# fgiral000/gencast-flax-nnx

Hardware: AMD Instinct MI355X
Metric: denoiser-calls/sec (higher is better)
Workload: dtype f16x3 (every product = 3 fp16 MFMAs on hi/lo-split f32 operands: 22-bit products, f32 accumulate; f32 storage); 1 GPU; nano-GenCast DPM-Solver++2S 20-step sample, 2.5deg grid (73x144), 1 ensemble member per GPU, batch 1; dead_call_skipped=True, grid_nodes=10512, mesh_nodes=2562, latent=256, layers=16, heads=4, ffw_hidden=2048, c_in=262, c_out=82, k_hop=8, parallelism=ensemble-dp1, broadcast=none, rccl_ranks=0, precision=f16x3, library_built_from_this_tree=True, launcher=single

## Files before the change

### gencast-flax-nnx_amd/csrc/gc_api.hip

```cpp
#include <dlfcn.h>

#include "gc_handle.h"

using namespace gci;

namespace {

void protect_pending_noise(gc_handle* h) {
  if (h->guard_pending && h->d_noise == h->last_noise) std::swap(h->d_noise, h->d_noise_alt);
}

int check_ready(gc_handle* h) {
  if (!h) return GC_ERR_INVALID_ARGUMENT;
  if (!h->finalized) return fail(h, GC_ERR_STATE, "gc_finalize has not been called");
  return GC_OK;
}

struct Rccl {
  void* lib = nullptr;
  ncclResult_t (*GetUniqueId)(ncclUniqueId*) = nullptr;
  ncclResult_t (*CommInitRank)(ncclComm_t*, int, ncclUniqueId, int) = nullptr;
  ncclResult_t (*CommDestroy)(ncclComm_t) = nullptr;
  ncclResult_t (*CommCount)(const ncclComm_t, int*) = nullptr;
  ncclResult_t (*CommUserRank)(const ncclComm_t, int*) = nullptr;
// ... 2 lines not shown
  const char* (*GetErrorString)(ncclResult_t) = nullptr;
  std::string error;
};

Rccl& rccl() {
  static Rccl r = [] {
    Rccl x;
    const char* override_path = std::getenv("GC_RCCL_LIBRARY");
    for (const char* name : {override_path ? override_path : "/opt/rocm/lib/librccl.so.1", "librccl.so.1", "librccl.so"}) {
      x.lib = dlopen(name, RTLD_NOW | RTLD_GLOBAL);
      if (x.lib) break;
    }
    if (!x.lib) {
      x.error = std::string("cannot load librccl: ") + dlerror();
      return x;
    }
    auto sym = [&](const char* n) {
      void* p = dlsym(x.lib, n);
      if (!p && x.error.empty()) x.error = std::string("librccl lacks ") + n;
      return p;
    };
    x.GetUniqueId = reinterpret_cast<decltype(x.GetUniqueId)>(sym("ncclGetUniqueId"));
    x.CommInitRank = reinterpret_cast<decltype(x.CommInitRank)>(sym("ncclCommInitRank"));
    x.CommDestroy = reinterpret_cast<decltype(x.CommDestroy)>(sym("ncclCommDestroy"));
    x.CommCount = reinterpret_cast<decltype(x.CommCount)>(sym("ncclCommCount"));
    x.CommUserRank = reinterpret_cast<decltype(x.CommUserRank)>(sym("ncclCommUserRank"));
    x.Broadcast = reinterpret_cast<decltype(x.Broadcast)>(sym("ncclBroadcast"));
    x.AllReduce = reinterpret_cast<decltype(x.AllReduce)>(sym("ncclAllReduce"));
    x.GetErrorString = reinterpret_cast<decltype(x.GetErrorString)>(sym("ncclGetErrorString"));
    return x;
  }();
  return r;
}

#define GC_NCCL(h, call)                                                                    \
  do {                                                                                      \
    ncclResult_t r__ = (call);                                                              \
    if (r__ != ncclSuccess) {                                                               \
      (h)->err = std::string(#call) + ": " + rccl().GetErrorString(r__);                    \
      return GC_ERR_COMM;                                                                   \
    }                                                                                       \
  } while (0)

}

static void destroy_impl(gc_handle* h);

extern "C" {

int gc_abi_version(void) { return GC_ABI_VERSION; }

const char* gc_build_info(void) {
#ifndef GC_SOURCE_HASH
#define GC_SOURCE_HASH "unknown"
#endif
  return "libgencast_hip gfx950 f16x3/f32-mfma " __DATE__ " " __TIME__ " src:" GC_SOURCE_HASH;
}

int gc_device_count(void) {
  int n = 0;
  if (hipGetDeviceCount(&n) != hipSuccess) return 0;
  return n;
}

int gc_device_pci_bus_id(int32_t device_id, char* out, int64_t cap) {
  if (!out || cap < 16 || device_id < 0 || device_id >= gc_device_count()) return GC_ERR_INVALID_ARGUMENT;
  out[0] = 0;
  return hipDeviceGetPCIBusId(out, (int)cap, device_id) == hipSuccess ? GC_OK : GC_ERR_HIP;
}

const char* gc_last_error(const gc_handle* h) { return h ? h->err.c_str() : g_create_error.c_str(); }

static void read_switches(gc_handle* h) {
  auto is = [](const char* name, const char* value) { const char* v = std::getenv(name); return v && std::string(v) == value; };
  auto off = [](const char* name) { const char* v = std::getenv(name); return v && *v && std::atoi(v) == 0; };
  auto on = [](const char* name) { const char* v = std::getenv(name); return v && *v == '1'; };
  h->f16x3 = !is("GC_PRECISION", "f32");
  h->use_graphs = !is("GC_TUNE_GRAPH", "0");
  h->m2g_fuse_sum = !off("GC_TUNE_M2G_FUSE_SUM");
  h->embed_cache = !off("GC_TUNE_EMBED_CACHE");
  h->attn_items = !off("GC_TUNE_ATTN_ITEMS");
  h->mlp_pair = !off("GC_TUNE_MLP_PAIR");
  h->edge_terms = !off("GC_TUNE_EDGE_TERMS");
  h->a16 = !off("GC_TUNE_A16");
  h->graph_serialize = on("GC_TUNE_GRAPH_SERIALIZE");
  h->graph_verbose = on("GC_TUNE_GRAPH_VERBOSE");
}

int gc_create(const gc_config* cfg, int device_id, gc_handle** out) {
  return guarded(nullptr, [&]() -> int {
  if (!cfg || !out) { g_create_error = "null argument"; return GC_ERR_INVALID_ARGUMENT; }
  *out = nullptr;
  const gc_config& c = *cfg;
  auto bad = [&](const char* m) { g_create_error = m; return GC_ERR_INVALID_ARGUMENT; };
  if (c.latent_size <= 0 || c.d_model <= 0 || c.num_heads <= 0 || c.ffw_hidden <= 0 ||
      c.num_layers < 0 || c.c_in <= 0 || c.c_out <= 0 || c.batch <= 0)
    return bad("all dimensions must be positive");
  if (c.c_out > c.c_in) return bad("c_out cannot exceed c_in (noisy targets are part of the forcings)");
  if (c.latent_size != c.d_model) return bad("latent_size must equal d_model");
  if (c.d_model % c.num_heads) return bad("num_heads has to divide d_model exactly");
  if (c.noise_num_frequencies <= 0 || c.noise_num_frequencies > 128 || c.noise_hidden <= 0 ||
      c.noise_hidden > 128 || !(c.noise_base_period > 0))
    return bad("noise encoder sizes out of range");
  auto unsup = [&](const char* m) { g_create_error = m; return GC_ERR_UNSUPPORTED; };
  if (c.latent_size != 128 && c.latent_size != 256 && c.latent_size != 512)
    return unsup("latent_size must be 128, 256 or 512 (MFMA column tiling)");
  const int dh = c.d_model / c.num_heads;
  if (dh != 32 && dh != 64 && dh != 128) return unsup("head size must be 32, 64 or 128");
  if (c.num_heads > 8) return unsup("at most 8 heads");
  if (c.ffw_hidden % 128) return unsup("ffw_hidden must be a multiple of 128");
  if (c.c_out > 512) return unsup("c_out must be <= 512");
  int ndev = 0;
  if (hipGetDeviceCount(&ndev) != hipSuccess || ndev == 0) {
    g_create_error = "no HIP device visible (this library has no CPU fallback)";
    return GC_ERR_NO_DEVICE;
  }
  if (device_id < 0 || device_id >= ndev) { g_create_error = "device_id out of range"; return GC_ERR_NO_DEVICE; }
  std::unique_ptr<gc_handle> h(new gc_handle());
  h->cfg = c;
  h->device = device_id;
  hipError_t e = hipSetDevice(device_id);
  if (e == hipSuccess) e = hipStreamCreateWithFlags(&h->stream, hipStreamNonBlocking);
  if (e == hipSuccess) e = hipStreamCreateWithFlags(&h->stream2, hipStreamNonBlocking);
  if (e == hipSuccess) e = hipEventCreate(&h->ev0);
  if (e == hipSuccess) e = hipEventCreate(&h->ev1);
  if (e == hipSuccess) e = hipEventCreateWithFlags(&h->ev_pin, hipEventDisableTiming);
  if (e == hipSuccess) e = hipMalloc((void**)&h->d_nonfinite, sizeof(unsigned));
  if (e == hipSuccess) e = hipMemset(h->d_nonfinite, 0, sizeof(unsigned));
  if (e == hipSuccess) e = hipHostMalloc((void**)&h->h_nonfinite, sizeof(unsigned), hipHostMallocDefault);
  if (e != hipSuccess) {
    g_create_error = hipGetErrorString(e);
    gc_destroy(h.release());
    return GC_ERR_HIP;
  }
  *h->h_nonfinite = 0;
  h->kp = round_up(3 + c.c_in, 32);
  read_switches(h.get());
  build_specs(h.get());
  *out = h.release();
  return GC_OK;
  });
}

void gc_destroy(gc_handle* h) {
  if (!h) return;
  try {
    destroy_impl(h);
  } catch (...) {
  }
}

static void destroy_impl(gc_handle* h) {
  (void)hipSetDevice(h->device);
  if (h->stream) (void)hipStreamSynchronize(h->stream);
  drop_sample_graphs(h);
  if (h->comm) (void)rccl().CommDestroy(h->comm);
  for (gc_handle::CtxSlot& c : h->ctx) {
    if (c.saved) (void)hipEventSynchronize(c.ev_w);
    if (c.read) (void)hipEventSynchronize(c.ev_r);
  }
  for (BufferGroup* g : h->groups) g->free();
  if (h->d_nonfinite) (void)hipFree(h->d_nonfinite);
  for (void* p : {(void*)h->h_nonfinite, (void*)h->pin_cond, (void*)h->pin_noise, (void*)h->pin_forc,
                  (void*)h->pin_lguard})
    if (p) (void)hipHostFree(p);
  if (h->ev_pin) (void)hipEventDestroy(h->ev_pin);
// ... 556 lines not shown
  GC_HIP(h, hipStreamSynchronize(h->stream));
  if (cls >= 0 && h->prof_events.empty()) {
    h->prof_events.resize(2 * 4096);
    for (auto& e : h->prof_events) GC_HIP(h, hipEventCreate(&e));
  }
  h->prof_cls = cls;
  h->prof_used = 0;
  return GC_OK;
}

int gc_profile_set_stride(gc_handle* h, int stride) {
  return guarded(h, [&]() -> int {
  if (!h) return GC_ERR_INVALID_ARGUMENT;
  if (stride < 1) return fail(h, GC_ERR_INVALID_ARGUMENT, "stride must be >= 1");
  h->prof_stride = stride;
  h->prof_seen = 0;
  return GC_OK;
  });
}

int gc_profile_read(gc_handle* h, int32_t* launches, float* total_ms) {
  return guarded(h, [&]() -> int {
  if (!h || !launches || !total_ms) return GC_ERR_INVALID_ARGUMENT;
  GC_HIP(h, hipSetDevice(h->device));
  GC_HIP(h, hipStreamSynchronize(h->stream));
  float tot = 0.f;
  for (size_t i = 0; i + 1 < h->prof_used; i += 2) {
    float ms = 0.f;
    GC_HIP(h, hipEventElapsedTime(&ms, h->prof_events[i], h->prof_events[i + 1]));
    tot += ms;
  }
  *launches = (int32_t)(h->prof_used / 2);
  *total_ms = tot;
  h->prof_used = 0;
  return GC_OK;
  });
}

int gc_algorithmic_work(gc_handle* h, double* flops, double* bytes) {
  return guarded(h, [&]() -> int {
  if (!h || !flops || !bytes) return GC_ERR_INVALID_ARGUMENT;
  if (!h->has_graph) return fail(h, GC_ERR_STATE, "gc_set_graph must be called first");
  const gc_config& c = h->cfg;
  const double B = c.batch, G = h->hg.G * B, M = h->hg.M * B, E1 = h->hg.E1 * B, E2 = h->hg.E2 * B;
  const double L = c.latent_size, D = c.d_model, F = c.ffw_hidden, NL = c.num_layers;
  const double nnz = (double)h->hg.khop_nnz * B;
  double f = 0;
  f += 2 * G * (3 + c.c_in) * L + 2 * G * L * L;
  f += 2 * E1 * 3 * L * L + 2 * E1 * L * L;
  f += 2 * M * 2 * L * L + 2 * M * L * L;
  f += 2 * G * L * L * 2;
  f += NL * (2 * M * D * 3 * D + 2 * M * D * D + 2 * M * D * F * 2 + 4 * nnz * D);
  f += 2 * E2 * 3 * L * L + 2 * E2 * L * L;
  f += 2 * G * 2 * L * L + 2 * G * L * L;
  f += 2 * G * L * L + 2 * G * L * c.c_out;
  f += (h->hidden_layers - 1) * 2.0 * L * L * (G + E1 + M + G + E2 + G + G);
  double params = 0;
  for (const auto& kv : h->specs) {
    double n = 1;
    for (auto d : kv.second) n *= (double)d;
    params += n;
  }
  *bytes = 4.0 * (params + G * (c.c_in + c.c_out) + 2 * G * L + NL * M * D * 10);
  *flops = f;
  return GC_OK;
  });
}

int gc_get_counter(gc_handle* h, const char* name, int64_t* value) {
  return guarded(h, [&]() -> int {
  if (!h) return GC_ERR_INVALID_ARGUMENT;
  if (!name || !value) return fail(h, GC_ERR_INVALID_ARGUMENT, "null argument");
  const std::string n(name);
  if (n == "range_fallbacks") *value = h->range_fallbacks;
  else if (n == "static_embedding_fallbacks") *value = h->static_embedding_fallbacks;
  else if (n == "launches_per_call") *value = h->launches_last_call;
  else if (n == "weights_f16_unsafe") *value = h->weights_f16_unsafe ? 1 : 0;
  else if (n == "fp16_storage") *value = h->last_route.st16 ? 1 : 0;
  else if (n == "split_edge") *value = h->split_edge ? 1 : 0;
  else if (n == "attention_items") *value = h->last_route.att_items;
  else if (n == "m2g_fused_sum") *value = h->last_route.m2g_fused ? 1 : 0;
  else if (n == "embed_cache") *value = h->embed_cache_samples;
  else if (n == "edge_term_samples") *value = h->edge_term_samples;
  else if (n == "edge_term_cache_bytes") *value = h->terms.ready ? h->terms.bytes : 0;
  else if (n == "graph_replays") *value = h->graph_replays;
  else if (n == "graph_captures") *value = h->graph_captures;
  else if (n == "loss_evaluations") *value = h->loss_evaluations;
  else if (n == "loss_device_us") *value = h->loss_device_us;
  else if (n == "ens_scores") *value = h->ens_scores;
  else if (n == "ens_score_device_us") *value = h->ens_score_device_us;
  else if (n == "ens_invalid_points") *value = h->ens_invalid_points;
  else if (n == "spec_calls") *value = h->spec_calls;
  else if (n == "spec_device_us") *value = h->spec_device_us;
  else if (n == "spec_invalid_columns") *value = h->spec_invalid_columns;
  else if (n == "ens_event_calls") *value = h->evt_calls;
  else if (n == "ens_event_device_us") *value = h->evt_device_us;
  else if (n == "ens_event_invalid_points") *value = h->evt_invalid_points;
  else if (n == "ens_derive_calls") *value = h->drv_calls;
  else if (n == "ens_derive_device_us") *value = h->drv_device_us;
  else if (n == "ens_order_calls") *value = h->ord_calls;
  else if (n == "ens_order_device_us") *value = h->ord_device_us;
  else if (n == "ens_order_invalid_points") *value = h->ord_invalid_points;
  else if (n == "ens_clim_calls") *value = h->clim_calls;
  else if (n == "ens_clim_device_us") *value = h->clim_device_us;
  else if (n == "ens_clim_invalid_points") *value = h->clim_invalid_points;
  else if (n == "ens_energy_calls") *value = h->en_calls;
  else if (n == "ens_energy_device_us") *value = h->en_device_us;
  else if (n == "ens_energy_invalid_points") *value = h->en_invalid_points;
  else if (n == "ens_variogram_calls") *value = h->vg_calls;
  else if (n == "ens_variogram_device_us") *value = h->vg_device_us;
  else if (n == "ens_tail_calls") *value = h->tail_calls;
  else if (n == "ens_tail_device_us") *value = h->tail_device_us;
  else if (n == "ens_tail_invalid_points") *value = h->tail_invalid_points;
  else if (n == "ens_region_calls") *value = h->reg_calls;
  else if (n == "ens_region_device_us") *value = h->reg_device_us;
  else if (n == "ens_feature_calls") *value = h->feat_calls;
  else if (n == "ens_feature_device_us") *value = h->feat_device_us;
  else if (n == "ens_region_invalid_points") *value = h->reg_invalid_points;
  else if (n == "ens_fss_calls") *value = h->fss_calls;
  else if (n == "ens_fss_device_us") *value = h->fss_device_us;
  else if (n == "ens_window_pushes") *value = h->win_pushes;
  else if (n == "ens_window_emits") *value = h->win_emits;
  else if (n == "ens_window_device_us") *value = h->win_device_us;
  else if (n == "ens_window_ring_bytes")
    *value = (int64_t)((size_t)h->win_ring_L * (((size_t)(h->win_ring_M + 1) * h->hg.G * h->cfg.batch * h->cfg.c_out + 3) / 4 * 4) * sizeof(float));
  else if (n == "noise_stream") *value = (int64_t)h->nz_stream;
  else if (n == "device_allocations") {
    *value = 0;
    for (const BufferGroup* g : h->groups) *value += (int64_t)g->ptrs.size();
  }
  else return fail(h, GC_ERR_INVALID_ARGUMENT, "unknown counter: " + n);
  return GC_OK;
  });
}

int gc_noise_set_tables(gc_handle* h, int32_t n_lat, int32_t n_lon, int32_t lmax, const float* legendre,
                        const float* cos_table, const float* sin_table) {
  return guarded(h, [&]() -> int {
  if (!h) return GC_ERR_INVALID_ARGUMENT;
  if (!h->has_graph) return fail(h, GC_ERR_STATE, "gc_set_graph must be called first");
  if (!legendre || !cos_table || !sin_table) return fail(h, GC_ERR_INVALID_ARGUMENT, "null argument");
  if (n_lat < 2 || n_lon < 2 || lmax < 1 || (int64_t)n_lat * n_lon != h->hg.G)
    return fail(h, GC_ERR_INVALID_ARGUMENT, "n_lat * n_lon must equal the number of grid nodes");
  const int N = h->cfg.batch * h->cfg.c_out;
  GC_HIP(h, hipSetDevice(h->device));
  int rc;
  const size_t L = (size_t)lmax;
  if ((rc = dev_upload(h, &h->d_nz_leg, std::vector<float>(legendre, legendre + L * n_lat * L)))) return rc;
  if ((rc = dev_upload(h, &h->d_nz_cos, std::vector<float>(cos_table, cos_table + (size_t)n_lon * L)))) return rc;
  if ((rc = dev_upload(h, &h->d_nz_sin, std::vector<float>(sin_table, sin_table + (size_t)n_lon * L)))) return rc;
  if ((rc = dev_alloc(h, &h->d_nz_coef, 2 * L * L * N + 4))) return rc;
  if ((rc = dev_alloc(h, &h->d_nz_f, 2 * L * n_lat * N))) return rc;
  h->nz_L = lmax; h->nz_lat = n_lat; h->nz_lon = n_lon;
  return GC_OK;
  });
}

int gc_noise_seed(gc_handle* h, uint64_t seed, uint64_t stream) {
  return guarded(h, [&]() -> int {
  if (!h) return GC_ERR_INVALID_ARGUMENT;
  if (h->guard_pending) {
    GC_HIP(h, hipSetDevice(h->device));
    int rc = resolve_guard(h);
    if (rc) return rc;
  }
  h->nz_key = seed;
// ... 465 lines not shown
```

### gencast-flax-nnx_amd/csrc/gc_forward.hip

```cpp
#include "gc_handle.h"

namespace gci {

template <class To, class From>
static const To& a16_view(const From& v) {
  static_assert(sizeof(To) == sizeof(From), "argument struct mismatch between the two kernel builds");
  return reinterpret_cast<const To&>(v);
}

Route make_route(const gc_handle* h) {
  const int D = h->cfg.d_model, F = h->cfg.ffw_hidden;
  Route r;
  r.f16 = h->f16x3 && !h->weights_f16_unsafe && !h->in_fallback;
  r.x32 = !r.f16 && h->f32_ws;
  const bool streams = r.f16 || r.x32;
  r.ffw_slabs = streams ? h->ffw_fused_slabs : 0;
  r.st16 = h->feat16 && h->a16 && r.f16 && D % 128 == 0 && D <= 512 &&
           (h->ffw_fused_slabs > 0 || (F % 128 == 0 && (F / h->ffw2_splits) % 128 == 0));
  r.v2 = r.f16 && r.ws(3 * D, D, 1);
  r.att_items = (h->att_n_items > 0 && r.ws(3 * D, D, 1) && h->attn_splits == 1 && D <= 512) ? h->att_n_items : 0;
  r.fuse_row = streams && D % 128 == 0 && D <= 512;
  r.node_ws = r.f16;
  r.split_edge = h->split_edge;
  r.try_pair = h->mlp_pair && h->hidden_layers == 1;
  r.m2g_fused = h->m2g_fuse_sum && h->hg.m2g_tri && h->hidden_layers == 1 && streams;
  r.embed_cache = h->embed_cache_live && h->embed_cache_ready && !h->feat16 && h->hidden_layers == 1 && streams;
  r.edge_terms = h->embed_cache_live && h->terms.ready && edge_terms_possible(h) && r.f16;
  return r;
}

bool edge_terms_possible(const gc_handle* h) {
  return h->edge_terms && h->f16x3 && !h->weights_f16_unsafe && !h->in_fallback && !h->feat16 && h->hidden_layers == 1 &&
         h->cfg.latent_size == 256 && h->cfg.batch == 1 && h->hg.m2g_tri;
}

static gc::Segment seg(const float* ptr, const int* index, const float* affine, int width, int ld, int bcast) {
  gc::Segment s;
  s.ptr = ptr; s.index = index; s.affine = affine; s.width = width; s.ld = ld; s.bcast = bcast;
  return s;
}

struct MlpCall {
  gc::Segment seg[3] = {};
  gc::AddTerm add[3] = {};
  int nseg = 0, nadd = 0, rows = 0, B = 1, ldo = 0;
  bool ln = true, cond = true;
  const float* residual = nullptr;
  float* out = nullptr;
  bool round_out = true;
  bool seg0_f32 = false, out_f32 = false;
  bool tri = false;
  MlpCall& segments(std::initializer_list<gc::Segment> l) { for (const auto& s : l) seg[nseg++] = s; return *this; }
  MlpCall& add_terms(std::initializer_list<gc::AddTerm> l) { for (const auto& t : l) add[nadd++] = t; return *this; }
};
static MlpCall mlp_call(std::initializer_list<gc::Segment> segs, int rows, int B, float* out, int ldo,
                        const float* residual = nullptr) {
  MlpCall c;
  c.rows = rows; c.B = B; c.out = out; c.ldo = ldo; c.residual = residual;
  return c.segments(segs);
}

static int build_mlp_args(gc_handle* h, const DevMlp& w, const MlpCall& c, gc::MlpArgs* out_args) {
  const Route& r = h->route;
  gc::MlpArgs& a = *out_args;
  a = gc::MlpArgs{};
  a.nseg = c.nseg; a.nadd = c.nadd;
  std::copy(c.seg, c.seg + c.nseg, a.seg);
  std::copy(c.add, c.add + c.nadd, a.add);
  a.rows = c.rows; a.B = c.B; a.hidden = h->cfg.latent_size;
  a.f16 = r.f16 ? 1 : 0;
  const Weight& w1 = c.nadd ? w.w1e : w.w1;
  a.w1t = pick(w1, r, Form::Staged); a.ldw1 = w1.ld; a.b1 = w.b1;
  a.w2t = pick(w.w2, r, Form::Staged); a.b2 = w.b2;
  if (r.f16 || r.x32) {
    a.w1f = pick(w1, r, Form::Streaming); a.k1f = w1.kf;
    a.w2f = pick(w.w2, r, Form::Streaming); a.ones = h->d_ones; a.zeros = h->d_zeros;
    a.f32w = r.x32 ? 1 : 0;
  }
  a.n_out = w.n_out; a.n_out_pad = w.n_out_pad; a.do_ln = c.ln ? 1 : 0;
  a.cond = (c.cond && w.cond_off >= 0) ? (h->cond_cur ? h->cond_cur : h->d_cond) + w.cond_off : nullptr;
  a.cond_stride = h->cond_total;
  a.residual = c.residual; a.out = c.out; a.ldo = c.ldo;
  a.round16 = h->feat16 ? 1 : 0;
  a.round_out = (h->feat16 && c.round_out) ? 1 : 0;
  a.a16 = r.st16 ? 1 : 0;
  a.seg0_f32 = c.seg0_f32 ? 1 : 0;
  a.out_f32 = c.out_f32 ? 1 : 0;
  a.tri = c.tri ? 1 : 0;
  if (c.tri && !gc::mlp_runs_weight_streaming(a))
    return fail(h, GC_ERR_INTERNAL, "the triple-sum epilogue exists in the weight-streaming MLP kernel only");
  return GC_OK;
}

static int enqueue_mlp(gc_handle* h, const gc::MlpArgs& a) {
  return launch(h, gc::KC_MLP, [&] {
    return a.a16 ? gc_a16::launch_mlp(h->stream, a16_view<gc_a16::MlpArgs>(a)) : gc::launch_mlp(h->stream, a);
  });
}
static int enqueue_mlp_pair(gc_handle* h, const gc::MlpArgs& a, const gc::MlpArgs& b) {
  return launch(h, gc::KC_MLP, [&] {
    return a.a16 ? gc_a16::launch_mlp_pair(h->stream, a16_view<gc_a16::MlpArgs>(a), a16_view<gc_a16::MlpArgs>(b))
                 : gc::launch_mlp_pair(h->stream, a, b);
  });
}
static int enqueue_gemm_ws(gc_handle* h, int cls, const gc::GemmArgs& ga, int mt, int splits, int epi) {
  return launch(h, cls, [&] {
    return ga.a16 ? gc_a16::launch_gemm_ws(h->stream, cls, a16_view<gc_a16::GemmArgs>(ga), mt, splits, epi)
                  : gc::launch_gemm_ws(h->stream, cls, ga, mt, splits, epi);
  });
}
static int enqueue_gemm_rowop(gc_handle* h, int cls, const gc::GemmArgs& ga, const gc::RowFuse& rf) {
  return launch(h, cls, [&] {
    return ga.a16 ? gc_a16::launch_gemm_rowop(h->stream, cls, a16_view<gc_a16::GemmArgs>(ga), a16_view<gc_a16::RowFuse>(rf))
                  : gc::launch_gemm_rowop(h->stream, cls, ga, rf);
  });
}
static int enqueue_ffw_fused(gc_handle* h, const gc::FfwArgs& fa) {
  return launch(h, gc::KC_GEMM_FFW1, [&] {
    return fa.a16 ? gc_a16::launch_ffw_fused(h->stream, a16_view<gc_a16::FfwArgs>(fa)) : gc::launch_ffw_fused(h->stream, fa);
  });
}

static int run_mlp_one(gc_handle* h, const DevMlp& w, const MlpCall& c) {
  gc::MlpArgs a{};
  if (int rc = build_mlp_args(h, w, c, &a)) return rc;
  return enqueue_mlp(h, a);
}

static int run_mlp(gc_handle* h, const DevMlp& w, const MlpCall& c) {
  if (w.pre.empty()) return run_mlp_one(h, w, c);
  if (c.nadd || c.tri || !h->d_mlp_tmp[0]) return fail(h, GC_ERR_INTERNAL, "hidden_layers >= 2: unsupported MLP form");
  const int L = h->cfg.latent_size;
  auto handed = [&](MlpCall m, size_t buf) {
    m.nseg = 0; m.seg0_f32 = true;
    return m.segments({seg(h->d_mlp_tmp[buf & 1], nullptr, nullptr, L, L, 0)});
  };
  MlpCall lead = c;
  lead.ln = lead.cond = lead.round_out = false; lead.residual = nullptr; lead.ldo = L; lead.out_f32 = true;
  for (size_t i = 0; i < w.pre.size(); ++i) {
    lead.out = h->d_mlp_tmp[i & 1];
    if (int rc = run_mlp_one(h, w.pre[i], i ? handed(lead, i - 1) : lead)) return rc;
  }
  return run_mlp_one(h, w, handed(c, w.pre.size() - 1));
}

int pick_ws_mt(int rows, int n, int splits) {
  const int panels = (n / 128) * splits;
  return ((rows + 63) / 64) * panels >= 400 ? 2 : 1;
}

bool build_attention_items(const gc::HostGraph& g, std::vector<int>* items, std::vector<int>* tiles) {
  const int n = g.n_tiles;
  tiles->assign((size_t)2 * n, 0);
  std::vector<std::vector<int>> lists(8);
  int slot = 0, any_cut = 0;
  for (int x = 0; x < 8; ++x) {
    const int t0 = (int)((long long)n * x / 8), t1 = (int)((long long)n * (x + 1) / 8), ng = t1 - t0;
    if (ng < 32) return false;
    if (ng >= 64) return false;
    const int n_cut = ng % 32;
    if (n_cut > 16) return false;
    any_cut += n_cut;
    std::vector<char> cut(ng, 0);
    for (int k = 0; k < n_cut; ++k) cut[(int)(((2LL * k + 1) * ng) / (2LL * n_cut))] = 1;
    std::vector<int>& it = lists[x];
    std::vector<int> order;
    for (int i = 0; i < ng; ++i) {
      const int t = t0 + i;
      if (cut[i]) { order.push_back(t); continue; }
      it.insert(it.end(), {t, g.tile_chunk_start[t], g.tile_chunk_start[t + 1], -1});
    }
// ... 80 lines not shown

static gc::GemmArgs mesh_gemm_args(const gc_handle* h, const float* a, int lda, bool ws) {
  gc::GemmArgs ga{};
  ga.a = a; ga.lda = lda; ga.a_f32 = 1; ga.rows = h->hg.M * h->cfg.batch;
  ga.round16 = h->feat16 ? 1 : 0; ga.a16 = h->route.st16 ? 1 : 0; ga.f32w = (ws && h->route.x32) ? 1 : 0;
  return ga;
}
static void merge_attention_partials(const gc_handle* h, gc::GemmArgs* ga) {
  const int D = h->cfg.d_model, H = h->cfg.num_heads;
  ga->att_po = h->d_apart_o; ga->att_pml = h->d_apart_ml; ga->att_B = h->cfg.batch; ga->att_H = H; ga->att_DH = D / H;
  if (h->attn_splits > 1) ga->att_S = h->attn_splits;
  else ga->att_tiles = h->d_att_tiles;
}
static int mesh_gemm(gc_handle* h, int cls, const float* a, int lda, const Weight& w, int n, int k, int splits,
                     const float* bias, int act, float* out, int ldo, int epi, bool att_merge = false) {
  const Route& r = h->route;
  const bool ws = r.ws(n, k, splits);
  gc::GemmArgs ga = mesh_gemm_args(h, a, lda, ws);
  ga.wt = pick(w, r, ws ? Form::Streaming : Form::Staged); ga.ldw = k; ga.n = n; ga.k_slice = k / splits;
  ga.bias = bias; ga.act = act; ga.out = out; ga.ldo = ldo;
  if (att_merge) merge_attention_partials(h, &ga);
  if (ws) return enqueue_gemm_ws(h, cls, ga, att_merge ? 1 : pick_ws_mt(ga.rows, n, splits), splits, epi);
  return launch(h, cls, [&] { return gc::launch_gemm(h->stream, cls, ga, splits, epi, r.f16); });
}

int forward(gc_handle* h, float sigma_scalar, const float* cond_ready) {
  const gc_config& c = h->cfg;
  const gc::HostGraph& g = h->hg;
  const int B = c.batch, L = c.latent_size, D = c.d_model, F = c.ffw_hidden;
  hipStream_t s = h->stream;
  int rc;
  const float* cond = cond_ready ? cond_ready : h->d_cond;
  h->cond_cur = cond;
  const int cs = h->cond_total;
  const int64_t launches0 = h->launch_count;
  const Route& r = h->route = h->last_route = make_route(h);

  if (!cond_ready && (rc = launch(h, gc::KC_COND, [&] {
         return gc::launch_cond(s, sigma_scalar < 0 ? h->d_sigma : nullptr, sigma_scalar, B, h->d_nw0t,
                                h->d_nb0, h->d_nw1t, h->d_nb1, c.noise_num_frequencies, c.noise_hidden,
                                c.noise_base_period, h->d_wc_all, h->d_bc_all, cs, h->d_condvec,
                                h->d_cond);
       })))
    return rc;

  {
    MlpCall embed = r.embed_cache ? mlp_call({seg(h->d_xn, nullptr, nullptr, h->nwp, h->nwp, 0)}, g.G * B, B, h->d_g0, L)
                                  : mlp_call({seg(h->d_xp, nullptr, nullptr, h->kp, h->kp, 0)}, g.G * B, B, h->d_g0, L);
    embed.seg0_f32 = true;
    if (r.embed_cache) embed.add_terms({{h->d_pstat, nullptr}});
    if ((rc = run_mlp(h, r.embed_cache ? h->g2m_embed_grid_n : h->g2m_embed_grid, embed))) return rc;
  }
  const size_t ML = (size_t)g.M * L;
  if (r.edge_terms && (h->term_slot < 0 || !h->terms.ready))
    return fail(h, GC_ERR_INTERNAL, "edge terms: the forward has no slot of the cache");
  const float* const m0 = r.edge_terms ? h->terms.m0 + h->term_slot * ML : h->d_m0;
  h->m0_cur = m0;
  if (!r.edge_terms && (rc = launch(h, gc::KC_PACK, [&] {
         return gc::launch_affine_rows(s, h->d_m0_hat, cond + h->g2m_embed_mesh.cond_off, cs, g.M, B, L,
                                       h->d_m0, h->feat16, r.st16);
       })))
    return rc;
  if (r.edge_terms && (rc = node_gemm(h, h->d_g0, g.G * B, h->g2m_edge.w1snd, h->d_pg))) return rc;
  const MlpCall edge = r.edge_terms
                           ? edge_terms_call(h, h->terms.T1 + (size_t)h->term_slot * g.E1 * L, g.E1, h->d_g2m_snd, h->d_g2m_rcv,
                                             h->d_pg, h->terms.Pm + h->term_slot * ML, h->d_e1)
                           : edge_call(h, h->d_e0_hat, cond + h->g2m_embed_edge.cond_off, g.E1, h->d_g2m_snd, h->d_g2m_rcv,
                                       h->d_g0, h->d_m0, h->d_pg, h->d_pm, h->d_e1);
  const MlpCall node = mlp_call({seg(h->d_g0, nullptr, nullptr, L, L, 0)}, g.G * B, B, h->d_g1, L, h->d_g0);
  gc::MlpArgs ea{}, na{};
  bool paired = false;
  if (r.try_pair) {
    if ((rc = build_mlp_args(h, h->g2m_edge, edge, &ea)) || (rc = build_mlp_args(h, h->g2m_grid, node, &na))) return rc;
    paired = gc::mlp_pair_supported(ea, na);
  }
  if (r.split_edge && (rc = edge_node_products(h, h->g2m_edge, h->d_g0, g.G * B, h->d_pg, h->d_m0, g.M * B, h->d_pm)))
    return rc;
  if ((rc = paired ? enqueue_mlp_pair(h, ea, na) : run_mlp(h, h->g2m_edge, edge))) return rc;
  if ((rc = launch(h, gc::KC_SEGSUM, [&] {
         return gc::launch_segsum(s, h->d_e1, h->d_g2m_ptr, h->d_g2m_eid, g.M, g.E1, B, L, h->d_agg1, h->feat16, r.st16,
                                  h->g2m_agg_norm);
       })))
    return rc;
  if ((rc = run_mlp(h, h->g2m_mesh, mlp_call({seg(m0, nullptr, nullptr, L, L, 0), seg(h->d_agg1, nullptr, nullptr, L, L, 0)},
                                             g.M * B, B, h->d_x, L, m0))))
    return rc;
  if (!paired && (rc = run_mlp(h, h->g2m_grid, node))) return rc;

  const int MB = g.M * B;
  const int n_layers = (h->debug_layer_limit >= 0 && h->debug_layer_limit < c.num_layers)
                           ? h->debug_layer_limit : c.num_layers;
  const float* pend_bias = nullptr;
  int pend_slabs = 0;
  auto rowop = [&](const float* bias, int slabs, int cond_off, float* hout) {
    return launch(h, gc::KC_ROWOP, [&] {
      return gc::launch_rowop(s, h->d_x, bias, h->d_part, slabs, MB, D, B, cond + cond_off, cs, hout, 0, h->feat16, r.st16);
    });
  };
  auto stop_here = [&](int i, int phase) { return h->debug_stop_layer == i && h->debug_stop_phase == phase; };
  const int* att_items = r.att_items ? h->d_att_items : nullptr;
  for (int i = 0; i < n_layers; ++i) {
    const DevLayer& ly = h->layers[i];
    if ((rc = rowop(pend_bias, pend_slabs, ly.cond_attn, h->d_h))) return rc;
    if (stop_here(i, 0)) return GC_OK;
    if (r.v2) {
      gc::GemmArgs ga = mesh_gemm_args(h, h->d_h, D, true);
      ga.wt = pick(ly.wqkv, r, Form::Streaming); ga.ldw = D; ga.n = 3 * D; ga.k_slice = D;
      ga.out = h->d_qkv; ga.ldo = r.st16 ? D : 3 * D;
      ga.kv16 = h->d_kv16; ga.kv_d = D;
      if ((rc = enqueue_gemm_ws(h, gc::KC_GEMM_QKV, ga, pick_ws_mt(MB, 3 * D, 1), 1, 3))) return rc;
      if (stop_here(i, 1)) return GC_OK;
      if ((rc = launch(h, gc::KC_ATTN, [&] {
             return gc::launch_attention_v2(s, h->d_qkv, h->d_kv16, h->d_att, h->d_apart_o, h->d_apart_ml, g.M, B, D,
                                            c.num_heads, h->attn_splits, h->d_tile_start, h->d_union, h->d_mask,
                                            g.n_tiles, h->max_tile_chunks, h->feat16, r.st16, att_items, r.att_items);
           })))
        return rc;
    } else {
      if ((rc = mesh_gemm(h, gc::KC_GEMM_QKV, h->d_h, D, ly.wqkv, 3 * D, D, 1, nullptr, 0, h->d_qkv, 3 * D, 0))) return rc;
      if (stop_here(i, 1)) return GC_OK;
      if ((rc = launch(h, gc::KC_ATTN, [&] {
             return gc::launch_attention(s, h->d_qkv, h->d_att, h->d_apart_o, h->d_apart_ml, g.M, B, D,
                                         c.num_heads, h->attn_splits, false, h->d_tile_start, h->d_union,
                                         h->d_mask, g.n_tiles, h->feat16, att_items, r.att_items);
           })))
        return rc;
    }
    if (r.fuse_row) {
      gc::GemmArgs ga = mesh_gemm_args(h, h->d_att, D, true);
      ga.wt = pick(ly.wo, r, Form::Streaming); ga.ldw = D; ga.n = D; ga.k_slice = D;
      if (h->attn_splits > 1 || r.att_items) merge_attention_partials(h, &ga);
      gc::RowFuse rf{h->d_x, ly.bo, cond + ly.cond_ffw, cs, B, h->d_h, h->feat16 ? 1 : 0};
      if ((rc = enqueue_gemm_rowop(h, gc::KC_GEMM_OUT, ga, rf))) return rc;
    } else {
      if ((rc = mesh_gemm(h, gc::KC_GEMM_OUT, h->d_att, D, ly.wo, D, D, h->out_splits, nullptr, 0, h->d_part, D, 1, h->attn_splits > 1)))
        return rc;
      if ((rc = rowop(ly.bo, h->out_splits, ly.cond_ffw, h->d_h))) return rc;
    }
    if (stop_here(i, 2)) return GC_OK;
    if (r.ffw_slabs > 0) {
      gc::FfwArgs fa{h->d_h, MB, (int)D, (int)F, pick(ly.w1, r, Form::Streaming), ly.b1, pick(ly.w2, r, Form::Streaming),
                     h->d_part, h->feat16 ? 1 : 0, r.st16 ? 1 : 0};
      fa.f32w = r.x32 ? 1 : 0;
      if ((rc = enqueue_ffw_fused(h, fa))) return rc;
    } else {
      if ((rc = mesh_gemm(h, gc::KC_GEMM_FFW1, h->d_h, D, ly.w1, F, D, 1, ly.b1, 1, h->d_u, F, 0))) return rc;
      if ((rc = mesh_gemm(h, gc::KC_GEMM_FFW2, h->d_u, F, ly.w2, D, F, h->ffw2_splits, nullptr, 0, h->d_part, D, 1))) return rc;
    }
    pend_bias = ly.b2;
    pend_slabs = r.ffw_slabs > 0 ? r.ffw_slabs : h->ffw2_splits;
  }
  if ((rc = rowop(pend_bias, pend_slabs, h->cond_final, h->d_m2))) return rc;

  if ((r.split_edge || r.edge_terms) && (rc = edge_node_products(h, h->m2g_edge, h->d_m2, g.M * B, h->d_pm, h->d_g1, g.G * B, h->d_pg)))
    return rc;
  if ((rc = run_m2g_edge(h, cond, r.m2g_fused))) return rc;
  if (!r.m2g_fused && (rc = launch(h, gc::KC_SEGSUM, [&] {
         return gc::launch_segsum(s, h->d_f1, h->d_m2g_ptr, h->d_m2g_eid, g.G, g.E2, B, L, h->d_agg2, h->feat16, r.st16);
       })))
    return rc;
  if ((rc = run_mlp(h, h->m2g_grid, mlp_call({seg(h->d_g1, nullptr, nullptr, L, L, 0), seg(h->d_agg2, nullptr, nullptr, L, L, 0)},
                                             g.G * B, B, h->d_g2, L, h->d_g1))))
    return rc;
  MlpCall dec = mlp_call({seg(h->d_g2, nullptr, nullptr, L, L, 0)}, g.G * B, B, h->d_y, c.c_out);
  dec.ln = dec.cond = false; dec.out_f32 = true;
  if ((rc = run_mlp(h, h->m2g_dec, dec))) return rc;
  h->launches_last_call = h->launch_count - launches0;
  return GC_OK;
}

int compute_static_embeddings(gc_handle* h) {
  const gc::HostGraph& hg = h->hg;
  const int L = h->cfg.latent_size;
  const struct { const DevMlp& w; const float* in; int items; float* out; } embeds[] = {
      {h->g2m_embed_mesh, h->d_mesh_struct16, hg.M, h->d_m0_hat},
      {h->g2m_embed_edge, h->d_e1_struct16, hg.E1, h->d_e0_hat},
      {h->m2g_embed_edge, h->d_e2_struct16, hg.E2, h->d_f0_hat}};
  if (int rc = drop_edge_terms(h)) return rc;
  auto run = [&]() -> int {
    h->route = make_route(h);
    for (const auto& e : embeds) {
      MlpCall c = mlp_call({seg(e.in, nullptr, nullptr, 32, 32, 1)}, e.items, 1, e.out, L);
      c.cond = c.round_out = false; c.seg0_f32 = c.out_f32 = true;
      if (int rc = run_mlp(h, e.w, c)) return rc;
    }
    return GC_OK;
  };
  if (int rc = run()) return rc;
  GC_HIP(h, hipStreamSynchronize(h->stream));
  if (!h->route.f16 || h->feat16) return GC_OK;
  const unsigned before = *h->h_nonfinite;
  for (const auto& e : embeds)
    if (int rc = launch(h, gc::KC_PACK, [&] { return gc::launch_finite_check(h->stream, e.out, (size_t)e.items * L, h->d_nonfinite); }))
      return rc;
  GC_HIP(h, hipMemcpyAsync(h->h_nonfinite, h->d_nonfinite, sizeof(unsigned), hipMemcpyDeviceToHost, h->stream));
  GC_HIP(h, hipStreamSynchronize(h->stream));
  const unsigned hits = *h->h_nonfinite - before;
  if (!hits) return GC_OK;
  h->nonfinite_seen += hits;
  ++h->static_embedding_fallbacks;
  h->in_fallback = true;
  const int rc = run();
  h->in_fallback = false;
  if (rc) return rc;
  GC_HIP(h, hipStreamSynchronize(h->stream));
  return GC_OK;
}

int drop_edge_terms(gc_handle* h) {
  if (h->terms.sigmas.empty() && h->term_allocs.ptrs.empty()) return GC_OK;
  if (!h->term_allocs.ptrs.empty()) {
    GC_HIP(h, hipStreamSynchronize(h->stream));
    drop_sample_graphs(h);
    h->term_allocs.free();
  }
  h->terms = gc_handle::EdgeTerms{};
  h->term_slot = -1;
  return GC_OK;
}

int ensure_edge_terms(gc_handle* h, const std::vector<float>& call_sigma) {
  if (!edge_terms_possible(h)) return GC_OK;
  gc_handle::EdgeTerms& t = h->terms;
  if (t.sigmas.size() == call_sigma.size() &&
      !std::memcmp(t.sigmas.data(), call_sigma.data(), call_sigma.size() * sizeof(float)))
    return GC_OK;
  if (int rc = drop_edge_terms(h)) return rc;
  t.sigmas = call_sigma;
  std::vector<float> distinct;
  for (float sg : call_sigma) {
    size_t k = 0;
    while (k < distinct.size() && std::memcmp(&distinct[k], &sg, sizeof(float))) ++k;
    if (k == distinct.size()) distinct.push_back(sg);
    t.call_slot.push_back((int)k);
  }
  const gc::HostGraph& g = h->hg;
  const gc_config& c = h->cfg;
  const size_t L = c.latent_size, n = distinct.size();
  const size_t per_slot = ((size_t)g.E1 + g.E2 + 2 * (size_t)g.M) * L;
  t.bytes = (int64_t)(n * per_slot * sizeof(float));
  if (n == 0 || n > (size_t)gc::kMaxSigmaList || t.bytes > h->edge_term_cap_mb * (int64_t)(1 << 20) ||
      n * (size_t)c.batch * h->cond_total > h->cond_all_cap) {
    t.bytes = 0;
    return GC_OK;
  }
  int rc;
  BufferGroup* own = &h->term_allocs;
  if ((rc = dev_alloc(h, &t.T1, n * g.E1 * L, own)) || (rc = dev_alloc(h, &t.T2, n * g.E2 * L, own)) ||
      (rc = dev_alloc(h, &t.m0, n * g.M * L, own)) || (rc = dev_alloc(h, &t.Pm, n * g.M * L, own)))
// ... 31 lines not shown
```

### gencast-flax-nnx_amd/csrc/gc_handle.h

```cpp
#pragma once
#include <hip/hip_runtime.h>

#include <algorithm>
#include <array>
#include <cmath>
#include <cstdio>
#include <cstdlib>
#include <cstring>
#include <map>
#include <memory>
#include <mutex>
#include <string>
#include <vector>

#include <rccl/rccl.h>

#include "../../include/gencast_hip.h"
#include "../../include/gencast_hip_debug.h"
#include "gc_graph.h"
#include "gc_kernels.h"

namespace gci {

inline int round_up(int v, int m) { return (v + m - 1) / m * m; }

struct Route {
  bool f16 = false;
  bool x32 = false;
  bool st16 = false;
  int ffw_slabs = 0;
  bool v2 = false;
  int att_items = 0;
  bool fuse_row = false;
  bool node_ws = false;
  bool m2g_fused = false;
  bool split_edge = false;
  bool try_pair = false;
  bool embed_cache = false;
  bool edge_terms = false;
  bool ws(int n, int k, int splits) const { return (f16 || x32) && n % 128 == 0 && (k / splits) % 128 == 0; }
};

struct Weight {
  float* t = nullptr;
  float* s = nullptr;
  float* f = nullptr;
  float* x = nullptr;
  int ld = 0, kf = 0;
};
enum class Form { Staged, Streaming };
inline const float* pick(const Weight& w, const Route& r, Form form) {
  if (form == Form::Streaming) return r.x32 ? w.x : w.f;
  return r.f16 ? w.s : w.t;
}

struct DevMlp {
  Weight w1, w2;
  Weight w1e, w1snd, w1rcv;
  float *b1 = nullptr, *b2 = nullptr;
  int n_out = 0, n_out_pad = 0;
  int cond_off = -1;
  std::vector<DevMlp> pre;
};

struct DevLayer {
  Weight wqkv, wo, w1, w2;
  float *bo = nullptr, *b1 = nullptr, *b2 = nullptr;
  int cond_attn = -1, cond_ffw = -1;
};

struct BufferGroup {
  std::vector<void*> ptrs;
  explicit BufferGroup(std::vector<BufferGroup*>& of_handle) { of_handle.push_back(this); }
  BufferGroup(const BufferGroup&) = delete;
  void free() {
    for (void* p : ptrs) (void)hipFree(p);
    ptrs.clear();
  }
  hipError_t drop(hipStream_t s) {
    const hipError_t e = hipStreamSynchronize(s);
    if (e == hipSuccess) free();
    return e;
  }
};

struct Event {
  hipEvent_t e = nullptr;
  explicit Event(std::vector<Event*>& of_handle) { of_handle.push_back(this); }
  Event(const Event&) = delete;
  hipError_t ensure(bool timing = false) {
    return e ? hipSuccess : timing ? hipEventCreate(&e) : hipEventCreateWithFlags(&e, hipEventDisableTiming);
  }
};

struct Bracket {
  Event e0, e1;
  explicit Bracket(std::vector<Event*>& of_handle) : e0(of_handle), e1(of_handle) {}
  hipError_t ensure() {
    const hipError_t e = e0.ensure(true);
    return e != hipSuccess ? e : e1.ensure(true);
  }
  hipError_t begin(hipStream_t s) { return hipEventRecord(e0.e, s); }
  hipError_t end(hipStream_t s) { return hipEventRecord(e1.e, s); }
  hipError_t microseconds(int64_t* us) {
    float ms = 0.f;
    const hipError_t e = hipEventElapsedTime(&ms, e0.e, e1.e);
    *us = (int64_t)(ms * 1000.0f);
    return e;
  }
};

}

struct gc_handle {
  std::vector<gci::BufferGroup*> groups;
  std::vector<gci::Event*> events;
  gc_config cfg{};
  int device = 0;
  hipStream_t stream = nullptr;
  hipStream_t stream2 = nullptr;
  std::string err;
  bool has_graph = false, finalized = false, has_slots = false, has_cond = false, has_noise = false;
  bool finalized_weights = false;
  gc::HostGraph hg;

  std::map<std::string, std::vector<int64_t>> specs;
  std::map<std::string, std::vector<float>> weights;
  gci::BufferGroup allocs{groups}, weight_allocs{groups}, cache_allocs{groups};

  int *d_g2m_snd = nullptr, *d_g2m_rcv = nullptr, *d_m2g_snd = nullptr, *d_m2g_rcv = nullptr;
  int *d_g2m_ptr = nullptr, *d_g2m_eid = nullptr, *d_m2g_ptr = nullptr, *d_m2g_eid = nullptr;
  int *d_tile_start = nullptr, *d_union = nullptr;
  int *d_att_items = nullptr, *d_att_tiles = nullptr;
  int att_n_items = 0;
  unsigned* d_mask = nullptr;
  float *d_grid_struct = nullptr, *d_mesh_struct16 = nullptr, *d_e1_struct16 = nullptr,
        *d_e2_struct16 = nullptr;

  gci::DevMlp g2m_embed_grid, g2m_embed_mesh, g2m_embed_edge, g2m_edge, g2m_mesh, g2m_grid;
  gci::DevMlp m2g_embed_edge, m2g_edge, m2g_grid, m2g_dec;
  std::vector<gci::DevLayer> layers;
  int cond_final = -1;
  int cond_total = 0;
  std::map<std::string, std::pair<int, int>> cond_sites;
  float *d_nw0t = nullptr, *d_nb0 = nullptr, *d_nw1t = nullptr, *d_nb1 = nullptr;
  float *d_wc_all = nullptr, *d_bc_all = nullptr;

  float *d_m0_hat = nullptr, *d_e0_hat = nullptr, *d_f0_hat = nullptr;

  int kp = 0;
  float *d_sigma = nullptr, *d_condvec = nullptr, *d_cond = nullptr;
  float* d_cond_all = nullptr;
  size_t cond_all_cap = 0;
  const float* cond_cur = nullptr;
  float *d_feats = nullptr, *d_xp = nullptr, *d_g0 = nullptr, *d_g1 = nullptr, *d_m0 = nullptr,
        *d_x = nullptr, *d_e1 = nullptr, *d_agg1 = nullptr, *d_qkv = nullptr, *d_att = nullptr,
        *d_u = nullptr, *d_m2 = nullptr, *d_f1 = nullptr, *d_agg2 = nullptr, *d_g2 = nullptr,
        *d_y = nullptr, *d_h = nullptr, *d_part = nullptr, *d_apart_o = nullptr, *d_apart_ml = nullptr,
        *d_pg = nullptr, *d_pm = nullptr;
  bool mlp_pair = true;
  bool embed_cache = true;
  bool embed_cache_ready = false;
  bool embed_cache_live = false;
  int nwp = 0;
  float *d_xn = nullptr, *d_pstat = nullptr;
  float *w1st_t = nullptr, *w1st_s = nullptr;
  gci::DevMlp g2m_embed_grid_n;
  std::vector<int> h_slots;
  int64_t embed_cache_samples = 0;
  bool m2g_fuse_sum = true;
  struct EdgeTerms {
    bool ready = false;
    std::vector<float> sigmas;
    std::vector<int> call_slot;
    float *T1 = nullptr, *T2 = nullptr, *m0 = nullptr, *Pm = nullptr;
    int64_t bytes = 0;
  };
  bool edge_terms = true;
  int64_t edge_term_cap_mb = 4096;
  EdgeTerms terms;
  gci::BufferGroup term_allocs{groups};
  int term_slot = -1;
  const float* m0_cur = nullptr;
  int64_t edge_term_samples = 0;
  float *d_ones = nullptr, *d_zeros = nullptr;
  int hidden_layers = 1;
  float* d_mlp_tmp[2] = {nullptr, nullptr};
  float *d_feats2 = nullptr, *d_ro_a = nullptr, *d_ro_b = nullptr, *d_ro_forc = nullptr;
  int *d_ro_kind = nullptr, *d_ro_src = nullptr, *d_ro_sidx = nullptr;
  int ro_nforc = -1, ro_forc_cap = 0;
  bool has_sample = false;
  int max_tile_chunks = 0;
  int ffw_fused_slabs = 0;
  void* d_kv16 = nullptr;
  bool f32_ws = true;
  bool split_edge = false;
  int attn_splits = 1, out_splits = 1, ffw2_splits = 1;
  gci::Route route;
  gci::Route last_route;
  bool a16 = true;
  bool attn_items = true;
  bool graph_serialize = false;
  bool graph_verbose = false;
  int* d_slots = nullptr;
  float *d_sx = nullptr, *d_sden = nullptr, *d_smid = nullptr, *d_noise = nullptr;
  float *d_noise_alt = nullptr, *last_noise = nullptr;
  float* d_stash = nullptr;
  hipEvent_t ev_stash = nullptr;
  bool has_stash = false;

  int nz_L = 0, nz_lat = 0, nz_lon = 0;
  float *d_nz_leg = nullptr, *d_nz_cos = nullptr, *d_nz_sin = nullptr, *d_nz_coef = nullptr, *d_nz_f = nullptr;
  unsigned long long nz_key = 0, nz_stream = 0;
  std::vector<float> churn_rates;
  float churn_inflation = 1.0f;

  bool has_loss_weights = false, has_targets = false, has_denoised = false;
  int loss_groups = 0;
  float *d_lw_node = nullptr, *d_lw_chan = nullptr, *d_lw_group = nullptr;
  int* d_l_group = nullptr;
  float *d_targets = nullptr, *d_lx = nullptr, *d_lden = nullptr;
  double* d_lpart = nullptr;
  float *d_lsig = nullptr, *d_lloss = nullptr, *d_lpg = nullptr;
  int loss_cap = 0;
  unsigned* pin_lguard = nullptr;
  int64_t loss_evaluations = 0, loss_device_us = 0;

  gci::BufferGroup ens_allocs{groups};
  int ens_members = 0;
  std::vector<char> ens_filled;
  float* d_ens = nullptr;
  double* d_ens_part = nullptr;
  unsigned* d_ens_hpart = nullptr;
  double* d_ens_sums = nullptr;
  unsigned long long* d_ens_hist = nullptr;
  float *d_ens_w = nullptr, *d_ens_truth = nullptr;
  float *d_ens_mean = nullptr, *d_ens_var = nullptr;
  bool has_ens_w = false, has_ens_truth = false, has_ens_fields = false;
  gci::Event ev_ens_free{events}, ev_ens_done{events};
  gci::Bracket ens_time{events};
  int64_t ens_scores = 0, ens_score_device_us = 0, ens_invalid_points = 0;
  std::vector<int32_t> ens_state_src;
  int* d_ens_state_src = nullptr;

  gci::BufferGroup ctx_allocs{groups};
  int ctx_slots = 0;
  float* d_ctx = nullptr;
  struct CtxSlot {
    bool saved = false;
    bool read = false;
    hipEvent_t ev_w = nullptr, ev_r = nullptr;
  };
  std::vector<CtxSlot> ctx;

  gci::BufferGroup spec_allocs{groups};
  gci::BufferGroup spec_work_allocs{groups};
  int sp_L = 0, sp_lat = 0, sp_lon = 0;
  int sp_sets = 0;
  float *d_sp_q = nullptr, *d_sp_tab = nullptr;
  float* d_sp_field = nullptr;
  double* d_sp_F = nullptr;
  double* d_sp_coef = nullptr;
  double* d_sp_out = nullptr;
  unsigned* d_sp_flags = nullptr;
  gci::Bracket spec_time{events};
  int64_t spec_calls = 0, spec_device_us = 0, spec_invalid_columns = 0;

// ... 73 lines not shown
  double* d_en_part = nullptr;
  unsigned* d_en_ipart = nullptr;
  double* d_en_out = nullptr;
  unsigned long long* d_en_outc = nullptr;
  gci::Bracket en_time{events};
  int64_t en_calls = 0, en_device_us = 0, en_invalid_points = 0;
  gci::BufferGroup vg_allocs{groups};
  bool vg_set = false;
  int vg_O = 0, vg_pk = 0, vg_n_lat = 0, vg_n_lon = 0;
  int* d_vg_offs = nullptr;
  double* d_vg_part = nullptr;
  unsigned* d_vg_cpart = nullptr;
  double* d_vg_out = nullptr;
  unsigned long long* d_vg_outc = nullptr;
  gci::Bracket vg_time{events};
  int64_t vg_calls = 0, vg_device_us = 0;

  gci::BufferGroup tail_allocs{groups};
  gci::BufferGroup tail_work_allocs{groups};
  int tail_T = 0;
  unsigned tail_dir_up = 0;
  int tail_work_T = 0;
  float* d_tail_thr = nullptr;
  double* d_tail_part = nullptr;
  unsigned* d_tail_cpart = nullptr;
  double* d_tail_out = nullptr;
  unsigned long long* d_tail_outc = nullptr;
  gci::Bracket tail_time{events};
  int64_t tail_calls = 0, tail_device_us = 0, tail_invalid_points = 0;

  gci::BufferGroup reg_allocs{groups};
  int reg_R = 0;
  int reg_listed = 0, reg_blocks = 0;
  std::vector<int> reg_plan;
  int reg_dev_M = 0;
  int* d_reg_plan = nullptr;
  double* d_reg_part = nullptr;
  unsigned* d_reg_hpart = nullptr;
  double* d_reg_sums = nullptr;
  unsigned long long* d_reg_hist = nullptr;
  gci::Bracket reg_time{events};
  int64_t reg_calls = 0, reg_device_us = 0, reg_invalid_points = 0;

  gci::BufferGroup feat_allocs{groups};
  gci::BufferGroup feat_work_allocs{groups};
  bool feat_set = false;
  bool feat_listed = false;
  int feat_c_src = 0, feat_n_lat = 0, feat_n_lon = 0, feat_max = 0, feat_list_M = 0;
  double* d_feat_depth = nullptr;
  int* d_feat_tab = nullptr;
  unsigned char* d_feat_work = nullptr;
  size_t feat_work_bytes = 0;
  int *d_feat_count = nullptr, *d_feat_node = nullptr;
  float* d_feat_value = nullptr;
  gci::Bracket feat_time{events};
  gci::Event ev_feat_src{events};
  int64_t feat_calls = 0, feat_device_us = 0;

  gci::BufferGroup fss_allocs{groups};
  gci::BufferGroup fss_work_allocs{groups};
  int fss_S = 0;
  int fss_n_lat = 0, fss_n_lon = 0;
  std::vector<int32_t> fss_rlat;
  int *d_fss_rlat = nullptr, *d_fss_rlon = nullptr;
  unsigned* d_fss_roww = nullptr;
  uint2* d_fss_work = nullptr;
  double* d_fss_part = nullptr;
  double* d_fss_out = nullptr;
  size_t fss_work_len = 0, fss_part_len = 0, fss_out_len = 0;
  gci::Bracket fss_time{events};
  int64_t fss_calls = 0, fss_device_us = 0;

  struct SampleGraph {
    std::vector<float> sigmas;
    int skip_dead = 1;
    const float* noise = nullptr;
    bool feat16 = false;
    gci::Route route;
    hipGraph_t graph = nullptr;
    hipGraphExec_t exec = nullptr, exec2 = nullptr;
    hipEvent_t done[2] = {nullptr, nullptr};
    int next = 0;
    int calls = 0;
    int64_t launches_per_call = 0, launches = 0;
    uint64_t last_use = 0;
  };
  bool use_graphs = true;
  std::vector<SampleGraph> sample_graphs;
  uint64_t graph_clock = 0;
  int64_t graph_replays = 0, graph_captures = 0;
  int debug_layer_limit = -1;
  int debug_stop_layer = -1, debug_stop_phase = -1;
  bool f16x3 = true;
  float g2m_agg_norm = 0.f;
  bool feat16 = false;
  bool weights_f16_unsafe = false;
  bool in_fallback = false;
  unsigned* d_nonfinite = nullptr;
  unsigned* h_nonfinite = nullptr;
  unsigned nonfinite_seen = 0;
  int64_t range_fallbacks = 0;
  int64_t static_embedding_fallbacks = 0;
  bool guard_pending = false;
  std::vector<float> last_sigmas;
  int last_skip_dead = 1;
  unsigned long long last_stream0 = 0;
  int64_t launches_last_call = 0, launch_count = 0;
  float *pin_cond = nullptr, *pin_noise = nullptr, *pin_forc = nullptr;
  size_t pin_forc_cap = 0;
  hipEvent_t ev_pin = nullptr;
  ncclComm_t comm = nullptr;
  int comm_rank = 0, comm_world = 1;
  double* d_comm_scalar = nullptr;

  int prof_cls = -1;
  int prof_stride = 1;
  unsigned prof_seen = 0;
  std::vector<hipEvent_t> prof_events;
  size_t prof_used = 0;
  hipEvent_t ev0 = nullptr, ev1 = nullptr;
};

namespace gci {

#define GC_HIP(h, call)                                                                     \
  do {                                                                                      \
    hipError_t e__ = (call);                                                                \
    if (e__ != hipSuccess) {                                                                \
      (h)->err = std::string(#call) + ": " + hipGetErrorString(e__);                        \
      return GC_ERR_HIP;                                                                    \
    }                                                                                       \
  } while (0)

inline int fail(gc_handle* h, int code, const std::string& msg) {
  h->err = msg;
  return code;
}

template <typename T>
int dev_alloc(gc_handle* h, T** p, size_t count, BufferGroup* owner = nullptr) {
  void* q = nullptr;
  GC_HIP(h, hipMalloc(&q, std::max<size_t>(count, 1) * sizeof(T)));
  (owner ? owner : &h->allocs)->ptrs.push_back(q);
  *p = reinterpret_cast<T*>(q);
  return GC_OK;
}

template <typename T>
int dev_upload(gc_handle* h, T** p, const std::vector<T>& v, BufferGroup* owner = nullptr) {
  int rc = dev_alloc(h, p, v.size(), owner);
  if (rc) return rc;
  if (!v.empty()) GC_HIP(h, hipMemcpy(*p, v.data(), v.size() * sizeof(T), hipMemcpyHostToDevice));
  return GC_OK;
}

template <typename F>
int launch(gc_handle* h, int cls, F&& f) {
  ++h->launch_count;
  bool prof = (h->prof_cls == cls) && (h->prof_used + 2 <= h->prof_events.size());
  if (prof && h->prof_stride > 1) prof = ((h->prof_seen++ % (unsigned)h->prof_stride) == 0);
  if (prof) GC_HIP(h, hipEventRecord(h->prof_events[h->prof_used], h->stream));
  hipError_t e = f();
  if (e != hipSuccess) {
    h->err = std::string("launch ") + gc::kernel_class_name(cls) + ": " + hipGetErrorString(e);
    return GC_ERR_HIP;
  }
  if (prof) {
// ... 71 lines not shown
```

### gencast-flax-nnx_amd/csrc/gc_kernels.hip

```cpp
#include "gc_kernels.h"

#include <algorithm>
#include <atomic>
#include <type_traits>

#include <math.h>
#include <stdlib.h>

#ifdef GC_TU_A16
#define GC_TU_NS gc_a16
#else
#define GC_TU_NS gc
#endif
namespace GC_TU_NS {
#ifdef GC_TU_A16
constexpr bool kTuA16 = true;
#else
constexpr bool kTuA16 = false;
#endif

#include "gc_dev_common.inc"


struct DynLdsOnce {
// ... 424 lines not shown
  return v;
}

template <int NT, int R>
__device__ __forceinline__ void ws_ring_fill(f32x4 (&wh)[R][NT], f32x4 (&wl)[R][NT], const float* wf,
                                             size_t ct_stride, int steps_total) {
#pragma unroll
  for (int j = 0; j < R; ++j) {
    const int sn = j < steps_total ? j : steps_total - 1;
#pragma unroll
    for (int nt = 0; nt < NT; ++nt) {
      wh[j][nt] = ld4(wf + nt * ct_stride + (size_t)sn * 512);
      wl[j][nt] = ld4(wf + nt * ct_stride + (size_t)sn * 512 + 256);
    }
  }
}

template <int MT, int NT, int R, int J0, bool A16 = false, bool F32 = false>
__device__ __forceinline__ void ws_quad(f32x16 (&acc)[MT][NT], f32x16 (&acc2)[MT][NT], f32x4 (&wh)[R][NT],
                                        f32x4 (&wl)[R][NT], const float* a_row, int mt_stride, int kstep0,
                                        const float* wf, size_t ct_stride, int& s, int steps_total) {
#pragma unroll
  for (int j = 0; j < 4; ++j) {
    const int kk = kstep0 + j;
    const int off = F32 ? kk * 16 : (kk >> 1) * 32 + (kk & 1) * 8;
#pragma unroll
    for (int mt = 0; mt < MT; ++mt) {
      if constexpr (F32) {
        const f32x4 a0 = ld4(a_row + mt * mt_stride + off), a1 = ld4(a_row + mt * mt_stride + off + 4);
#pragma unroll
        for (int e = 0; e < 4; ++e)
#pragma unroll
          for (int nt = 0; nt < NT; ++nt) acc[mt][nt] = mfma32(wh[J0 + j][nt][e], a0[e], acc[mt][nt]);
#pragma unroll
        for (int e = 0; e < 4; ++e)
#pragma unroll
          for (int nt = 0; nt < NT; ++nt) acc[mt][nt] = mfma32(wl[J0 + j][nt][e], a1[e], acc[mt][nt]);
        continue;
      }
      const f32x4 ah = ld4(a_row + mt * mt_stride + off);
      f32x4 al;
      if constexpr (!A16) al = ld4(a_row + mt * mt_stride + off + 16);
#pragma unroll
      for (int nt = 0; nt < NT; ++nt) acc2[mt][nt] = mfma16(wl[J0 + j][nt], ah, acc2[mt][nt]);
#pragma unroll
      for (int nt = 0; nt < NT; ++nt) acc[mt][nt] = mfma16(wh[J0 + j][nt], ah, acc[mt][nt]);
      if constexpr (!A16) {
#pragma unroll
        for (int nt = 0; nt < NT; ++nt) acc2[mt][nt] = mfma16(wh[J0 + j][nt], al, acc2[mt][nt]);
      }
    }
    __builtin_amdgcn_sched_barrier(0);
    int sn = s + R;
    if (sn >= steps_total) sn = steps_total - 1;
#pragma unroll
    for (int nt = 0; nt < NT; ++nt) {
      wh[J0 + j][nt] = ld4(wf + nt * ct_stride + (size_t)sn * 512);
      wl[J0 + j][nt] = ld4(wf + nt * ct_stride + (size_t)sn * 512 + 256);
    }
    ++s;
    __builtin_amdgcn_sched_barrier(0);
  }
}

__device__ __forceinline__ void ln_accumulate(const f32x4& y, float& s1, float& s2) {
#pragma unroll
  for (int e = 0; e < 4; ++e) {
    s1 += y[e];
    s2 = __builtin_fmaf(y[e], y[e], s2);
  }
}
__device__ __forceinline__ void ln_finish(float s1, float s2, float inv_n, float& mean, float& rstd) {
  mean = s1 * inv_n;
  const float var = fmaxf(__builtin_fmaf(-mean, mean, s2 * inv_n), 0.f);
  rstd = 1.0f / sqrtf(var + 1e-6f);
}
__device__ __forceinline__ f32x4 ln_affine(const f32x4& y, float mean, float rstd, const f32x4& sc, const f32x4& of) {
  f32x4 r;
#pragma unroll
  for (int e = 0; e < 4; ++e) r[e] = __builtin_fmaf((y[e] - mean) * rstd, sc[e], of[e]);
  return r;
}

template <int NT1, int WM, int NWC>
constexpr int mlp_ws_occ() { return NWC >= 8 ? (NT1 == 1 ? 4 : 2) : ((WM >= 2 || NT1 >= 4) ? 1 : 2); }
template <int NT1, int NT2, int MT, int WM, int NWC, int NW2, int OCC, bool A16, bool F32, bool TERMS = false>
__device__ __forceinline__ void gc_mlp_ws_body(const MlpArgs& a, const int bid) {
  static_assert(!(A16 && F32), "one or the other");
  static_assert(!TERMS || (!A16 && !F32 && (NT1 * 32 * NWC) % 256 == 0 && (32 * MT) % (4 * NWC) == 0), "terms form: f16x3, whole 1 KB rows per wave");
  extern __shared__ __attribute__((aligned(16))) float smem[];
  constexpr int HID = NT1 * 32 * NWC, NPAD = NT2 * 32 * NW2, BM = 32 * MT * WM, NTHR = 64 * NWC * WM;
  constexpr int KC = BM >= 128 ? 64 : 128, LDA = KC + 4, LDH = HID + 4, LDY = NPAD + 4;
  constexpr int PPR = KC / 4;
  constexpr int RSTEP = NTHR / PPR;
  constexpr int AP = BM / RSTEP;
  constexpr int R1 = (OCC < 4 && (NT1 * MT <= 2 || (NT1 >= 4 && MT == 1))) ? 8 : 4;
  constexpr int R2 = (OCC < 4 && (NT2 * MT <= 2 || (NT1 >= 4 && NT2 * MT <= 4))) ? 8 : 4;
  int* srcoff = reinterpret_cast<int*>(smem);
  int* srcb = srcoff + 3 * BM;
  int* addoff = srcb + BM;
  float* region = smem + 6 * BM;

  const int tid = threadIdx.x;
  const int wave_all = tid >> 6, lane = tid & 63, r = lane & 31, hh = lane >> 5;
  const int wave = wave_all % NWC, wrow = (wave_all / NWC) * (MT * 32);
  const int row0 = bid * BM;
  constexpr int TPB = BM / 3;
  const int tri = a.tri;
  const int unit0 = bid * TPB, units = a.rows / 3;
  const int w0 = a.seg[0].width, w1 = a.nseg > 1 ? a.seg[1].width : 0, w2 = a.nseg > 2 ? a.seg[2].width : 0;
  const int ktot = w0 + w1 + w2, kpad = a.k1f;

  const float *p0 = a.seg[0].ptr, *p1 = a.seg[1].ptr, *p2 = a.seg[2].ptr;
  const float *f0 = a.seg[0].affine, *f1 = a.nseg > 1 ? a.seg[1].affine : nullptr,
              *f2 = a.nseg > 2 ? a.seg[2].affine : nullptr;
  if constexpr (TERMS) {
    const int *ax0 = a.add[0].index, *ax1 = a.add[1].index, *ax2 = a.add[2].index;
    for (int idx = tid; idx < a.nadd * BM; idx += NTHR) {
      const int t = idx / BM, i = idx - t * BM;
      int grow = row0 + i;
      if (grow >= a.rows) grow = a.rows - 1;
      int item = grow / a.B, b = grow - item * a.B;
      if (tri) {
        const int j = i / 3;
        int u = unit0 + j;
        if (u >= units) u = units - 1;
        const int gi = u / a.B;
        b = u - gi * a.B;
        item = 3 * gi + (i - 3 * j);
      }
      const int* ax = pick3(t, ax0, ax1, ax2);
      srcoff[idx] = ((ax ? ax[item] : item) * a.B + b) * HID;
    }
  }
  if constexpr (!TERMS) {
    const int *ix0 = a.seg[0].index, *ix1 = a.seg[1].index, *ix2 = a.seg[2].index;
    const int bc0 = a.seg[0].bcast, bc1 = a.seg[1].bcast, bc2 = a.seg[2].bcast;
    const int ld0 = a.seg[0].ld, ld1 = a.seg[1].ld, ld2 = a.seg[2].ld;
    for (int idx = tid; idx < a.nseg * BM; idx += NTHR) {
      const int sgi = idx / BM, i = idx - sgi * BM;
      int grow = row0 + i;
      if (grow >= a.rows) grow = a.rows - 1;
      int item = grow / a.B, b = grow - item * a.B;
      if (tri) {
        const int j = i / 3;
        int u = unit0 + j;
        if (u >= units) u = units - 1;
        const int gi = u / a.B;
        b = u - gi * a.B;
        item = 3 * gi + (i - 3 * j);
      }
      const int* ix = pick3(sgi, ix0, ix1, ix2);
      const int bc = pick3(sgi, bc0, bc1, bc2);
      const int ld = pick3(sgi, ld0, ld1, ld2);
      int srow = ix ? ix[item] : item;
      if (!bc) srow = srow * a.B + b;
      srcoff[idx] = srow * ld;
      if (sgi == 0) srcb[i] = b;
    }
    const int* ax0 = a.add[0].index;
    const int* ax1 = a.add[1].index;
    for (int idx = tid; idx < a.nadd * BM; idx += NTHR) {
      const int t = idx / BM, i = idx - t * BM;
      int grow = row0 + i;
      if (grow >= a.rows) grow = a.rows - 1;
      int item = grow / a.B, b = grow - item * a.B;
      if (tri) {
        const int j = i / 3;
        int u = unit0 + j;
        if (u >= units) u = units - 1;
        const int gi = u / a.B;
// ... 279 lines not shown
        f32x4 y3[3][CG];
#pragma unroll
        for (int sl = 0; sl < 3; ++sl)
#pragma unroll
          for (int j = 0; j < CG; ++j) {
            const int c = 4 * lane + 256 * j;
            f32x4 y = {0.f, 0.f, 0.f, 0.f};
            if (c < NPAD) {
              y = ld4(Ybuf + (3 * jt + sl) * LDY + c);
#pragma unroll
              for (int e = 0; e < 4; ++e)
                if (c + e >= n) y[e] = 0.f;
            }
            y3[sl][j] = y;
          }
        float mean3[3] = {0.f, 0.f, 0.f}, rstd3[3] = {1.f, 1.f, 1.f};
        if (a.do_ln) {
          float s1[3], s2[3];
#pragma unroll
          for (int sl = 0; sl < 3; ++sl) {
            s1[sl] = 0.f;
            s2[sl] = 0.f;
#pragma unroll
            for (int j = 0; j < CG; ++j) ln_accumulate(y3[sl][j], s1[sl], s2[sl]);
          }
#pragma unroll
          for (int o = 32; o > 0; o >>= 1)
#pragma unroll
            for (int sl = 0; sl < 3; ++sl) {
              s1[sl] += __shfl_xor(s1[sl], o);
              s2[sl] += __shfl_xor(s2[sl], o);
            }
#pragma unroll
          for (int sl = 0; sl < 3; ++sl) ln_finish(s1[sl], s2[sl], inv_n, mean3[sl], rstd3[sl]);
        }
#pragma unroll
        for (int j = 0; j < CG; ++j) {
          const int c = 4 * lane + 256 * j;
          if (c >= n) continue;
          f32x4 sc = scpre[j], of = ofpre[j];
          if (a.cond && a.B != 1) {
            const float* cs = a.cond + (size_t)(u % a.B) * a.cond_stride;
            sc = ld4(cs + c);
            of = ld4(cs + n + c);
          }
          f32x4 t = r16_c<RND>(ln_affine(y3[0][j], mean3[0], rstd3[0], sc, of));
          t += r16_c<RND>(ln_affine(y3[1][j], mean3[1], rstd3[1], sc, of));
          t += r16_c<RND>(ln_affine(y3[2][j], mean3[2], rstd3[2], sc, of));
          t = r16_c<RND>(t);
          if (A16 && !a.out_f32) sth4(as_h16(a.out) + (size_t)u * a.ldo + c, t);
          else st4(a.out + (size_t)u * a.ldo + c, t);
        }
      }
    });
    return;
  }
#pragma unroll
  for (int j = 0; j < CG; ++j) {
    const int c = 4 * lane + 256 * j;
#pragma unroll
    for (int rr = 0; rr < RW; ++rr) {
      const int orow = row0 + rbase + rr;
      f32x4 rs = {0.f, 0.f, 0.f, 0.f};
      if (a.residual && orow < a.rows && c < n) {
        if constexpr (A16) {
          if (vec_io) {
            rs = ldh4(as_h16(a.residual) + (size_t)orow * n + c);
          } else {
#pragma unroll
            for (int e = 0; e < 4; ++e)
              if (c + e < n) rs[e] = (float)as_h16(a.residual)[(size_t)orow * n + c + e];
          }
        } else if (vec_io) {
          rs = ld4(a.residual + (size_t)orow * n + c);
        } else {
#pragma unroll
          for (int e = 0; e < 4; ++e)
            if (c + e < n) rs[e] = a.residual[(size_t)orow * n + c + e];
        }
      }
      rv[rr][j] = rs;
    }
  }
  __syncthreads();
#pragma unroll
  for (int rr = 0; rr < RW; ++rr) {
#pragma unroll
    for (int j = 0; j < CG; ++j) {
      const int c = 4 * lane + 256 * j;
      f32x4 y = {0.f, 0.f, 0.f, 0.f};
      if (c < NPAD) {
        y = ld4(Ybuf + (rbase + rr) * LDY + c);
#pragma unroll
        for (int e = 0; e < 4; ++e)
          if (c + e >= n) y[e] = 0.f;
      }
      yv[rr][j] = y;
    }
  }
  float mean[RW], rstd[RW];
  if (a.do_ln) {
    float s1[RW], s2[RW];
#pragma unroll
    for (int rr = 0; rr < RW; ++rr) {
      s1[rr] = 0.f;
      s2[rr] = 0.f;
#pragma unroll
      for (int j = 0; j < CG; ++j) ln_accumulate(yv[rr][j], s1[rr], s2[rr]);
    }
#pragma unroll
    for (int o = 32; o > 0; o >>= 1)
#pragma unroll
      for (int rr = 0; rr < RW; ++rr) {
        s1[rr] += __shfl_xor(s1[rr], o);
        s2[rr] += __shfl_xor(s2[rr], o);
      }
#pragma unroll
    for (int rr = 0; rr < RW; ++rr) ln_finish(s1[rr], s2[rr], inv_n, mean[rr], rstd[rr]);
  } else {
#pragma unroll
    for (int rr = 0; rr < RW; ++rr) {
      mean[rr] = 0.f;
      rstd[rr] = 1.f;
    }
  }
  with_flag(a.round_out, [&](auto rc) __attribute__((always_inline)) {
  constexpr bool RND = decltype(rc)::value;
#pragma unroll
  for (int j = 0; j < CG; ++j) {
    const int c = 4 * lane + 256 * j;
    if (c >= n) continue;
    const f32x4 sc1 = scpre[j], of1 = ofpre[j];
#pragma unroll
    for (int rr = 0; rr < RW; ++rr) {
      const int orow = row0 + rbase + rr;
      if (orow >= a.rows) break;
      f32x4 sc = sc1, of = of1;
      if (a.cond && !(a.B == 1 && vec_io)) {
        const float* cs = a.cond + (size_t)(orow % a.B) * a.cond_stride;
#pragma unroll
        for (int e = 0; e < 4; ++e)
          if (c + e < n) {
            sc[e] = cs[c + e];
            of[e] = cs[n + c + e];
          }
      }
      const f32x4 v = r16_c<RND>(r16_c<RND>(ln_affine(yv[rr][j], mean[rr], rstd[rr], sc, of)) + rv[rr][j]);
      if (A16 && !a.out_f32) {
        if (vec_io) {
          sth4(as_h16(a.out) + (size_t)orow * a.ldo + c, v);
        } else {
#pragma unroll
          for (int e = 0; e < 4; ++e)
            if (c + e < n) as_h16(a.out)[(size_t)orow * a.ldo + c + e] = (_Float16)v[e];
        }
      } else if (vec_io) {
        st4(a.out + (size_t)orow * a.ldo + c, v);
      } else {
#pragma unroll
        for (int e = 0; e < 4; ++e)
          if (c + e < n) a.out[(size_t)orow * a.ldo + c + e] = v[e];
      }
    }
  }
  });
}

template <int NT1, int NT2, int MT, int WM, int NWC = 4, int NW2 = NWC,
          int OCC = mlp_ws_occ<NT1, WM, NWC>() , bool A16 = false,
          bool F32 = false, bool TERMS = false>
__global__ __launch_bounds__(64 * NWC * WM, OCC) void gc_mlp_ws_kernel(MlpArgs a) {
  gc_mlp_ws_body<NT1, NT2, MT, WM, NWC, NW2, OCC, A16, F32, TERMS>(a, (int)blockIdx.x);
}

template <int NT1, int NT2, int MT, int WM, int NWC = 4, int NW2 = NWC,
          int OCC = mlp_ws_occ<NT1, WM, NWC>(), bool A16 = false, bool F32 = false, bool TERMS_A = false >
__global__ __launch_bounds__(64 * NWC * WM, OCC) void gc_mlp_ws_pair_kernel(MlpArgs a, MlpArgs b, int na) {
  if ((int)blockIdx.x < na) gc_mlp_ws_body<NT1, NT2, MT, WM, NWC, NW2, OCC, A16, F32, TERMS_A>(a, (int)blockIdx.x);
  else gc_mlp_ws_body<NT1, NT2, MT, WM, NWC, NW2, OCC, A16, F32>(b, (int)blockIdx.x - na);
}

template <int NT1, int NT2, int MT, int WM, int NWC, int NW2>
static hipError_t mlp_ws_geometry(const MlpArgs& a, int* grid_out, size_t* lds_out) {
  constexpr int HID = NT1 * 32 * NWC, NPAD = NT2 * 32 * NW2, BM = 32 * MT * WM;
  constexpr int abuf = 2 * BM * ((BM >= 128 ? 64 : 128) + 4);
  constexpr int region = (abuf > BM * (HID + 4)) ? abuf : BM * (HID + 4);
  static_assert(BM * (NPAD + 4) <= region, "output tile must fit the shared region");
  *lds_out = (size_t)(6 * BM + region) * sizeof(float);
  if (a.nadd < 0 || a.nadd > 3 || (a.nadd > 0 && !a.add[0].ptr) || (a.nadd > 1 && !a.add[1].ptr) || (a.nadd > 2 && !a.add[2].ptr))
    return hipErrorInvalidValue;
  if (a.nseg != 0 && a.nadd > 2) return hipErrorInvalidValue;
  int ksum = 0;
  for (int i = 0; i < a.nseg; ++i) {
    if (a.seg[i].width % 32 || a.seg[i].ld % 4) return hipErrorInvalidValue;
    ksum += a.seg[i].width;
  }
  if (a.nseg == 0) {
    if (a.nadd < 1 || !a.f16 || a.f32w || a.a16 || a.round16 || !a.w2f) return hipErrorInvalidValue;
  } else if (a.k1f % 64 || a.k1f < ksum || a.k1f - ksum >= 64 || !a.w2f || !a.ones || !a.zeros || ksum > 512 * 3) {
    return hipErrorInvalidValue;
  }
  if (kTuA16) {
    constexpr int KCc = BM >= 128 ? 64 : 128;
    for (int i = 0; i < a.nseg; ++i) {
      const bool h16 = !(i == 0 && a.seg0_f32);
      if (h16 && (a.seg[i].affine || a.seg[i].ld % 8 || a.seg[i].width % 8)) return hipErrorInvalidValue;
      if (a.nseg > 1 && a.seg[i].width % KCc) return hipErrorInvalidValue;
    }
  }
  int grid = (a.rows + BM - 1) / BM;
  if (a.tri) {
    if (a.rows % 3 || a.residual || a.ldo % 4 || a.n_out % 4 ||
        (a.cond && ((reinterpret_cast<size_t>(a.cond) & 15) || a.cond_stride % 4)))
      return hipErrorInvalidValue;
    grid = (a.rows / 3 + BM / 3 - 1) / (BM / 3);
  }
  *grid_out = grid;
  return hipSuccess;
}

template <int NT1, int NT2, int MT, int WM, int NWC = 4, int NW2 = NWC, bool TERMS_A = false>
static hipError_t launch_mlp_ws_pair_t(hipStream_t s, const MlpArgs& a, const MlpArgs& b) {
  int ga = 0, gb = 0;
  size_t lds = 0;
  if (hipError_t e = mlp_ws_geometry<NT1, NT2, MT, WM, NWC, NW2>(a, &ga, &lds)) return e;
  if (hipError_t e = mlp_ws_geometry<NT1, NT2, MT, WM, NWC, NW2>(b, &gb, &lds)) return e;
  constexpr int OCC = mlp_ws_occ<NT1, WM, NWC>();
  if ((a.nseg == 0) != TERMS_A || b.nseg == 0) return hipErrorInvalidValue;
  if constexpr (TERMS_A) {
    if constexpr (kTuA16) return hipErrorInvalidValue;
    else {
      static DynLdsOnce once_t;
      if (hipError_t e = once_t.ensure((const void*)gc_mlp_ws_pair_kernel<NT1, NT2, MT, WM, NWC, NW2, OCC, false, false, true>, (int)lds)) return e;
      hipLaunchKernelGGL((gc_mlp_ws_pair_kernel<NT1, NT2, MT, WM, NWC, NW2, OCC, false, false, true>), dim3(ga + gb),
                         dim3(64 * NWC * WM), lds, s, a, b, ga);
      return hipGetLastError();
    }
  }
  if constexpr (!kTuA16) {
    if (a.f32w) {
      static DynLdsOnce once32;
      if (hipError_t e = once32.ensure((const void*)gc_mlp_ws_pair_kernel<NT1, NT2, MT, WM, NWC, NW2, OCC, false, true>, (int)lds)) return e;
      hipLaunchKernelGGL((gc_mlp_ws_pair_kernel<NT1, NT2, MT, WM, NWC, NW2, OCC, false, true>), dim3(ga + gb),
                         dim3(64 * NWC * WM), lds, s, a, b, ga);
      return hipGetLastError();
    }
  }
  static DynLdsOnce once;
  if (hipError_t e = once.ensure((const void*)gc_mlp_ws_pair_kernel<NT1, NT2, MT, WM, NWC, NW2, OCC, kTuA16>, (int)lds)) return e;
  hipLaunchKernelGGL((gc_mlp_ws_pair_kernel<NT1, NT2, MT, WM, NWC, NW2, OCC, kTuA16>), dim3(ga + gb),
                     dim3(64 * NWC * WM), lds, s, a, b, ga);
  return hipGetLastError();
}

template <int NT1, int NT2, int MT, int WM, int NWC = 4, int NW2 = NWC, bool TERMS = false>
static hipError_t launch_mlp_ws_t(hipStream_t s, const MlpArgs& a) {
  int grid = 0;
  size_t lds = 0;
  if (hipError_t e = mlp_ws_geometry<NT1, NT2, MT, WM, NWC, NW2>(a, &grid, &lds)) return e;
  constexpr int OCC = mlp_ws_occ<NT1, WM, NWC>();
  if ((a.nseg == 0) != TERMS) return hipErrorInvalidValue;
  if constexpr (TERMS) {
    if constexpr (kTuA16) return hipErrorInvalidValue;
    else {
      static DynLdsOnce once_t;
      if (hipError_t e = once_t.ensure((const void*)gc_mlp_ws_kernel<NT1, NT2, MT, WM, NWC, NW2, OCC, false, false, true>, (int)lds)) return e;
      hipLaunchKernelGGL((gc_mlp_ws_kernel<NT1, NT2, MT, WM, NWC, NW2, OCC, false, false, true>), dim3(grid),
                         dim3(64 * NWC * WM), lds, s, a);
      return hipGetLastError();
    }
  }
  if constexpr (!kTuA16) {
    if (a.f32w) {
      static DynLdsOnce once32;
      if (hipError_t e = once32.ensure((const void*)gc_mlp_ws_kernel<NT1, NT2, MT, WM, NWC, NW2, OCC, false, true>, (int)lds)) return e;
      hipLaunchKernelGGL((gc_mlp_ws_kernel<NT1, NT2, MT, WM, NWC, NW2, OCC, false, true>), dim3(grid),
                         dim3(64 * NWC * WM), lds, s, a);
      return hipGetLastError();
    }
  }
  static DynLdsOnce once;
  if (hipError_t e = once.ensure((const void*)gc_mlp_ws_kernel<NT1, NT2, MT, WM, NWC, NW2, OCC, kTuA16>, (int)lds)) return e;
  hipLaunchKernelGGL((gc_mlp_ws_kernel<NT1, NT2, MT, WM, NWC, NW2, OCC, kTuA16>), dim3(grid),
                     dim3(64 * NWC * WM), lds, s, a);
  return hipGetLastError();
}

template <int NT1, int NT2, bool F16, int WM>
static hipError_t launch_mlp_t(hipStream_t s, const MlpArgs& a) {
  const int hidden = NT1 * 128, n_pad = NT2 * 128, bm = 32 * WM;
  const int wrows = hidden > n_pad ? hidden : n_pad;
  const size_t lds = (size_t)(wrows * kMlpLd + bm * kMlpLd + bm * (hidden + 4)) * sizeof(float);
  for (int i = 0; i < a.nseg; ++i)
    if (a.seg[i].width % kMlpBK || a.seg[i].ld % 4) return hipErrorInvalidValue;
  static DynLdsOnce once;
  if (hipError_t e = once.ensure((const void*)gc_mlp_kernel<NT1, NT2, F16, WM>, (int)lds)) return e;
  const int grid = (a.rows + bm - 1) / bm;
  hipLaunchKernelGGL((gc_mlp_kernel<NT1, NT2, F16, WM>), dim3(grid), dim3(256 * WM), lds, s, a);
  return hipGetLastError();
}

constexpr int kMlpMt2Rows = 24000;

bool mlp_runs_weight_streaming(const MlpArgs& a) {
  const int nt1 = a.hidden / 128, nt2 = a.n_out_pad / 128;
  if (a.hidden % 128 || a.n_out_pad % 128 || a.n_out_pad > a.hidden || !((a.f16 || a.f32w) && a.w1f)) return false;
  if (nt1 <= 2) return nt2 <= nt1;
  return nt1 == 4 && (nt2 == 4 || nt2 == 1);
}

hipError_t launch_mlp(hipStream_t s, const MlpArgs& a) {
  const int nt1 = a.hidden / 128, nt2 = a.n_out_pad / 128;
  if (a.hidden % 128 || a.n_out_pad % 128 || a.n_out_pad > a.hidden) return hipErrorInvalidValue;
  if (mlp_runs_weight_streaming(a)) {
    if (a.nseg == 0) {
      if (nt1 != 2 || nt2 != 2) return hipErrorInvalidValue;
      return a.rows >= kMlpMt2Rows ? launch_mlp_ws_t<2, 2, 2, 1, 4, 4, true>(s, a) : launch_mlp_ws_t<1, 1, 1, 1, 8, 8, true>(s, a);
    }
    if (nt1 == 4) return nt2 == 4 ? launch_mlp_ws_t<2, 2, 2, 1, 8, 8>(s, a) : launch_mlp_ws_t<2, 1, 2, 1, 8, 4>(s, a);
    const bool mt2 = a.rows >= kMlpMt2Rows;
    if (nt1 == 2 && !mt2) return nt2 == 2 ? launch_mlp_ws_t<1, 1, 1, 1, 8, 8>(s, a) : launch_mlp_ws_t<1, 1, 1, 1, 8, 4>(s, a);
    if (nt1 == 2) return nt2 == 2 ? launch_mlp_ws_t<2, 2, 2, 1>(s, a) : launch_mlp_ws_t<2, 1, 2, 1>(s, a);
    return mt2 ? launch_mlp_ws_t<1, 1, 2, 1>(s, a) : launch_mlp_ws_t<1, 1, 1, 1>(s, a);
  }
  if (a.f16 || a.a16 || a.tri || !a.w1t || a.nadd < 0 || a.nadd > 2 || a.nseg == 0) return hipErrorInvalidValue;
  for (int i = 0; i < a.nadd; ++i)
    if (!a.add[i].index) return hipErrorInvalidValue;
#define GC_MLP(A_, B_) \
  if (nt1 == A_ && nt2 == B_) return launch_mlp_t<A_, B_, false, 1>(s, a);
  GC_MLP(1, 1) GC_MLP(2, 2) GC_MLP(2, 1) GC_MLP(4, 4) GC_MLP(4, 1)
#undef GC_MLP
  return hipErrorInvalidValue;
}

bool mlp_pair_supported(const MlpArgs& a, const MlpArgs& b) {
  auto ok = [](const MlpArgs& m) {
    if (!mlp_runs_weight_streaming(m) || m.tri || m.n_out_pad != m.hidden) return false;
    return m.hidden == 512 || (m.hidden == 256 && m.rows < kMlpMt2Rows);
  };
  if (b.nseg == 0 || (a.nseg == 0 && a.hidden != 256)) return false;
  return ok(a) && ok(b) && a.hidden == b.hidden && a.f16 == b.f16 && a.f32w == b.f32w && a.a16 == b.a16;
}
hipError_t launch_mlp_pair(hipStream_t s, const MlpArgs& a, const MlpArgs& b) {
  if (!mlp_pair_supported(a, b)) return hipErrorInvalidValue;
  if (a.hidden == 512) return launch_mlp_ws_pair_t<2, 2, 2, 1, 8, 8>(s, a, b);
  if (a.nseg == 0) return launch_mlp_ws_pair_t<1, 1, 1, 1, 8, 8, true>(s, a, b);
  return launch_mlp_ws_pair_t<1, 1, 1, 1, 8, 8>(s, a, b);
}

template <bool H16>
__device__ __forceinline__ f32x4 seg_ld4(const float* base, size_t elem) {
  if constexpr (H16) return ldh4(as_h16(base) + elem);
  else return ld4(base + elem);
}
template <bool H16>
__device__ __forceinline__ void seg_st4(float* base, size_t elem, f32x4 v) {
  if constexpr (H16) sth4(as_h16(base) + elem, v);
  else st4(base + elem, v);
}

template <bool H16>
__global__ __launch_bounds__(256) void gc_segsum_kernel(const float* __restrict__ src,
                                                         const int* __restrict__ rowptr,
                                                         const int* __restrict__ eids, int n_items,
                                                         int B, int width, float* __restrict__ out, int round16,
                                                         float norm ) {
  __shared__ __attribute__((aligned(16))) float part[4][512];
  const int wrow = blockIdx.x;
  const int wave = threadIdx.x >> 6, lane = threadIdx.x & 63;
  const int item = wrow / B, b = wrow - item * B;
  const int e0 = rowptr[item], e1 = rowptr[item + 1];
  const int n_w = (e1 - e0 - wave + 3) >> 2;
  for (int c0 = 0; c0 < width; c0 += 256) {
    const int c = c0 + lane * 4;
    const int cc = c < width ? c : 0;
    f32x4 s0 = {0.f, 0.f, 0.f, 0.f}, s1 = {0.f, 0.f, 0.f, 0.f};
    for (int kb = 0; kb < n_w; kb += 64) {
      const int mine = e0 + wave + 4 * (kb + lane);
      const int id = eids[mine < e1 ? mine : e1 - 1];
      const int cnt = (n_w - kb) < 64 ? (n_w - kb) : 64;
      for (int j = 0; j < cnt; j += 8) {
        f32x4 v[8];
#pragma unroll
        for (int u = 0; u < 8; ++u) {
          const int ju = (j + u < cnt) ? j + u : cnt - 1;
          const int idj = __builtin_amdgcn_readlane(id, ju);
          v[u] = seg_ld4<H16>(src, ((size_t)idj * B + b) * width + cc);
        }
        __builtin_amdgcn_sched_barrier(0);
#pragma unroll
        for (int u = 0; u < 8; ++u)
          if (j + u < cnt) {
            if (u & 1) s1 += v[u];
            else s0 += v[u];
          }
      }
    }
    s0 += s1;
    if (c < width) st4(&part[wave][lane * 4], s0);
    __syncthreads();
    if (wave == 0 && c < width) {
      f32x4 t = ld4(&part[0][lane * 4]);
      t += ld4(&part[1][lane * 4]);
      t += ld4(&part[2][lane * 4]);
      t += ld4(&part[3][lane * 4]);
      if (norm != 0.f) t = t / norm;
      seg_st4<H16>(out, (size_t)wrow * width + c, r16_if(t, round16));
    }
    __syncthreads();
  }
}

template <bool H16>
__global__ __launch_bounds__(256) void gc_segsum_small_kernel(const float* __restrict__ src,
                                                               const int* __restrict__ rowptr,
                                                               const int* __restrict__ eids, int n_items,
                                                               int B, int width, float* __restrict__ out, int round16,
                                                               float norm) {
  const int wrow = blockIdx.x * 4 + (threadIdx.x >> 6);
  const int lane = threadIdx.x & 63;
  if (wrow >= n_items * B) return;
  const int item = wrow / B, b = wrow - item * B;
  const int e0 = rowptr[item], e1 = rowptr[item + 1];
  for (int c = lane * 4; c < width; c += 256) {
    f32x4 acc = {0.f, 0.f, 0.f, 0.f};
    for (int e = e0; e < e1; e += 4) {
      int id[4];
// ... 1343 lines not shown
      const int cbase = (wave * NT2 + nt) * 32 + 4 * hh;
#pragma unroll
      for (int j = 0; j < 4; ++j) {
        f32x4 v;
#pragma unroll
        for (int e = 0; e < 4; ++e) v[e] = hilo(acc2[mt][nt][4 * j + e], accx2[mt][nt][4 * j + e]);
        st4(orow + cbase + 8 * j, v);
      }
    }
  }
#ifdef GC_STAMPS
  GC_STAMP();
  asm volatile("s_waitcnt vmcnt(0)" ::: "memory");
  GC_STAMP();
  if (g.stamps && lane == 0)
    for (int i = 0; i < 8; ++i) g.stamps[((size_t)blockIdx.x * NWC + wave) * 8 + i] = stamp_v[i];
#endif
#undef GC_STAMP
}

template <int ND, int MT, int NWC = 4>
static hipError_t launch_ffw_fused_t(hipStream_t s, const FfwArgs& g) {
  const size_t lds = (size_t)(32 * MT * ((ND > 2 ? 128 * ND : 256) + 4)) * sizeof(float);
  const int grid = ((g.rows + 32 * MT - 1) / (32 * MT)) * (g.f / 256);
  if (grid <= 0) return hipSuccess;
  if constexpr (!kTuA16) {
    if (g.f32w) {
      static DynLdsOnce once32;
      if (hipError_t e = once32.ensure((const void*)gc_ffw_fused_kernel<ND, MT, NWC, false, true>, (int)lds)) return e;
      hipLaunchKernelGGL((gc_ffw_fused_kernel<ND, MT, NWC, false, true>), dim3(grid), dim3(64 * NWC), lds, s, g);
      return hipGetLastError();
    }
  }
  static DynLdsOnce once;
  if (hipError_t e = once.ensure((const void*)gc_ffw_fused_kernel<ND, MT, NWC, kTuA16>, (int)lds)) return e;
  hipLaunchKernelGGL((gc_ffw_fused_kernel<ND, MT, NWC, kTuA16>), dim3(grid), dim3(64 * NWC), lds, s, g);
  return hipGetLastError();
}

hipError_t launch_ffw_fused(hipStream_t s, const FfwArgs& g) {
  if ((g.d != 128 && g.d != 256) || g.f % 256 || g.f < 256) return hipErrorInvalidValue;
  const bool big = ((g.rows + 63) / 64) * (g.f / 256) >= 300;
  if (g.d == 128) return big ? launch_ffw_fused_t<1, 2>(s, g) : launch_ffw_fused_t<1, 1>(s, g);
  const int b96 = ((g.rows + 95) / 96) * (g.f / 256);
  if (b96 > 128 && b96 <= 256) return launch_ffw_fused_t<2, 3, 8>(s, g);
  return big ? launch_ffw_fused_t<2, 2>(s, g) : launch_ffw_fused_t<2, 1>(s, g);
}

hipError_t launch_gemm_ws(hipStream_t s, int cls, const GemmArgs& g, int mt, int splits, int epi) {
  switch (cls) {
    case KC_GEMM_QKV: return launch_gemm_ws_c<KC_GEMM_QKV>(s, g, mt, splits, epi);
    case KC_GEMM_OUT: return launch_gemm_ws_c<KC_GEMM_OUT>(s, g, mt, splits, epi);
    case KC_GEMM_FFW1: return launch_gemm_ws_c<KC_GEMM_FFW1>(s, g, mt, splits, epi);
    case KC_GEMM_FFW2: return launch_gemm_ws_c<KC_GEMM_FFW2>(s, g, mt, splits, epi);
    case KC_GEMM_NODE: return launch_gemm_ws_c<KC_GEMM_NODE>(s, g, mt, splits, epi);
    default: return hipErrorInvalidValue;
  }
}

hipError_t launch_gemm(hipStream_t s, int cls, const GemmArgs& g, int splits, int epi, bool f16) {
  switch (cls) {
    case KC_GEMM_QKV: return launch_gemm_c<KC_GEMM_QKV>(s, g, splits, epi, f16);
    case KC_GEMM_OUT: return launch_gemm_c<KC_GEMM_OUT>(s, g, splits, epi, f16);
    case KC_GEMM_FFW1: return launch_gemm_c<KC_GEMM_FFW1>(s, g, splits, epi, f16);
    case KC_GEMM_FFW2: return launch_gemm_c<KC_GEMM_FFW2>(s, g, splits, epi, f16);
    case KC_GEMM_NODE: return launch_gemm_c<KC_GEMM_NODE>(s, g, splits, epi, f16);
    default: return hipErrorInvalidValue;
  }
}

template <int NS , bool H16 = false>
__global__ __launch_bounds__(256) void gc_rowop_kernel(float* __restrict__ x,
                                                        const float* __restrict__ bias,
                                                        const float* __restrict__ partials, int n_slabs,
                                                        int rows, int d, int B,
                                                        const float* __restrict__ cond, int cond_stride,
                                                        float* __restrict__ h, int h_s16, int round16) {
  const int row = blockIdx.x * 4 + (threadIdx.x >> 6);
  const int lane = threadIdx.x & 63;
  if (row >= rows) return;
  const size_t slab = (size_t)rows * d;
  const float* cs = cond + (size_t)(row % B) * cond_stride;
  float4 v[2], scv[2], ofv[2];
  float s1 = 0.f, s2 = 0.f;
  const float4 zero4 = make_float4(0.f, 0.f, 0.f, 0.f);
#pragma unroll
  for (int i = 0; i < 2; ++i) {
    const int c = 4 * lane + 256 * i;
    v[i] = zero4; scv[i] = zero4; ofv[i] = zero4;
    if (c < d) {
      const float* pr = partials + (size_t)row * d + c;
      float4 p[NS > 0 ? NS : 1];
      if constexpr (NS > 0) {
#pragma unroll
        for (int j = 0; j < NS; ++j) p[j] = *reinterpret_cast<const float4*>(pr + (size_t)j * slab);
      }
      float4 a;
      if constexpr (H16) {
        const f32x4 xa = ldh4(as_h16(x) + (size_t)row * d + c);
        a = make_float4(xa[0], xa[1], xa[2], xa[3]);
      } else {
        a = *reinterpret_cast<const float4*>(x + (size_t)row * d + c);
      }
      float4 bb = zero4;
      if (bias) bb = *reinterpret_cast<const float4*>(bias + c);
      if (h) {
        scv[i] = *reinterpret_cast<const float4*>(cs + c);
        ofv[i] = *reinterpret_cast<const float4*>(cs + d + c);
      }
      if constexpr (NS > 0) {
        a.x += bb.x; a.y += bb.y; a.z += bb.z; a.w += bb.w;
#pragma unroll
        for (int j = 0; j < NS; ++j) { a.x += p[j].x; a.y += p[j].y; a.z += p[j].z; a.w += p[j].w; }
      } else {
        a.x += bb.x; a.y += bb.y; a.z += bb.z; a.w += bb.w;
        for (int sidx = 0; sidx < n_slabs; ++sidx) {
          const float4 q = *reinterpret_cast<const float4*>(pr + (size_t)sidx * slab);
          a.x += q.x; a.y += q.y; a.z += q.z; a.w += q.w;
        }
      }
      if (round16) { a.x = r16(a.x); a.y = r16(a.y); a.z = r16(a.z); a.w = r16(a.w); }
      if (n_slabs > 0 || bias) {
        if constexpr (H16) sth4(as_h16(x) + (size_t)row * d + c, f32x4{a.x, a.y, a.z, a.w});
        else *reinterpret_cast<float4*>(x + (size_t)row * d + c) = a;
      }
      v[i] = a;
      s1 += a.x + a.y + a.z + a.w;
      s2 += a.x * a.x + a.y * a.y + a.z * a.z + a.w * a.w;
    }
  }
  if (!h) return;
  s1 = wave_sum(s1);
  s2 = wave_sum(s2);
  const float mean = s1 / (float)d;
  const float var = fmaxf(s2 / (float)d - mean * mean, 0.f);
  const float rstd = 1.0f / sqrtf(var + 1e-6f);
#pragma unroll
  for (int i = 0; i < 2; ++i) {
    const int c = 4 * lane + 256 * i;
    if (c < d) {
      const float4 sc = scv[i];
      const float4 of = ofv[i];
      float4 o;
      o.x = (v[i].x - mean) * rstd * sc.x + of.x;
      o.y = (v[i].y - mean) * rstd * sc.y + of.y;
      o.z = (v[i].z - mean) * rstd * sc.z + of.z;
      o.w = (v[i].w - mean) * rstd * sc.w + of.w;
      if (round16) { o.x = r16(o.x); o.y = r16(o.y); o.z = r16(o.z); o.w = r16(o.w); }
      if constexpr (H16) sth4(as_h16(h) + (size_t)row * d + c, f32x4{o.x, o.y, o.z, o.w});
      else if (h_s16) store4_s16(h, (size_t)row, d, c, o.x, o.y, o.z, o.w);
      else *reinterpret_cast<float4*>(h + (size_t)row * d + c) = o;
    }
  }
}

hipError_t launch_rowop(hipStream_t s, float* x, const float* bias, const float* partials, int n_slabs,
                        int rows, int d, int B, const float* cond, int cond_stride, float* h, int h_s16,
                        bool round16, bool h16) {
  if (d > 512 || d % 4 || h_s16 < 0 || h_s16 > 1 || (h_s16 && d % 32) || (h16 && h_s16 == 1)) return hipErrorInvalidValue;
  const int n_blocks = (rows + 3) / 4;
#define GC_ROWOP_NS(NS_)                                                                                   \
  if (h16) hipLaunchKernelGGL((gc_rowop_kernel<NS_, true>), dim3(n_blocks), dim3(256), 0, s, x, bias, partials, n_slabs, \
                     rows, d, B, cond, cond_stride, h, h_s16, 1);                           \
  else hipLaunchKernelGGL((gc_rowop_kernel<NS_, false>), dim3(n_blocks), dim3(256), 0, s, x, bias, partials, n_slabs, \
                     rows, d, B, cond, cond_stride, h, h_s16, round16 ? 1 : 0)
  switch (n_slabs) {
    case 1: GC_ROWOP_NS(1); break;
    case 2: GC_ROWOP_NS(2); break;
    case 4: GC_ROWOP_NS(4); break;
    case 8: GC_ROWOP_NS(8); break;
    default: GC_ROWOP_NS(-1); break;
  }
#undef GC_ROWOP_NS
  return hipGetLastError();
}

template <int DH>
__global__ __launch_bounds__(DH >= 128 ? 256 : 512) void gc_attention_kernel(
    const float* __restrict__ qkv, float* __restrict__ o, float* __restrict__ part_o,
    float* __restrict__ part_ml, int M, int B, int D, int S, int out_s16,
    const int* __restrict__ tile_chunk_start, const int* __restrict__ union_idx,
    const unsigned* __restrict__ mask_bits, int feat16, const int* __restrict__ items, int n_items) {
  constexpr int HK = DH / 2;
  constexpr int NS = DH / 32;
  int t = blockIdx.x, sp = blockIdx.y, it_lo = 0, it_hi = 0, it_slot = -1;
  const int b = blockIdx.z;
  if (items) {
    const int xcd = blockIdx.x & 7, jj = blockIdx.x >> 3;
    const int lin = xcd * (n_items >> 3) + jj;
    t = items[4 * lin];
    if (t < 0) return;
    it_lo = items[4 * lin + 1]; it_hi = items[4 * lin + 2]; it_slot = items[4 * lin + 3];
    sp = 0;
  }
  const int head = threadIdx.x >> 6, H = blockDim.x >> 6;
  const int lane = threadIdx.x & 63, r = lane & 31, hh = lane >> 5;
  const size_t ld = (size_t)3 * D;
  const float scale = 1.0f / sqrtf((float)DH);
  const float kNegBig = -1e30f;
  const float kThr = feat16 ? 10.0f : 40.0f;

  int qnode = t * kTileM + r;
  if (qnode >= M) qnode = M - 1;
  float qf[HK];
  {
    const float* qp = qkv + ((size_t)qnode * B + b) * ld + head * DH + hh * HK;
#pragma unroll
    for (int i = 0; i < HK; i += 4) {
      const float4 v = *reinterpret_cast<const float4*>(qp + i);
      qf[i] = v.x * scale;
      qf[i + 1] = v.y * scale;
      qf[i + 2] = v.z * scale;
      qf[i + 3] = v.w * scale;
    }
  }
  f32x16 oacc[NS];
#pragma unroll
  for (int sl = 0; sl < NS; ++sl)
#pragma unroll
    for (int g = 0; g < 16; ++g) oacc[sl][g] = 0.f;
  float m_run = kNegBig, l_run = 0.f;

  int lo, hi;
  if (items) {
    lo = it_lo;
    hi = it_hi;
  } else {
    const int c_begin = tile_chunk_start[t], nc = tile_chunk_start[t + 1] - c_begin;
    lo = c_begin + (nc * sp) / S;
    hi = c_begin + (nc * (sp + 1)) / S;
  }
  const float* kbase = qkv + (size_t)b * ld + D + head * DH + hh * HK;
  const float* vbase = qkv + (size_t)b * ld + 2 * D + head * DH + r;

// ... 512 lines not shown
  } else if (dh == 32) GC_ATT2F(32)
  else if (dh == 64) GC_ATT2F(64)
  else GC_ATT2F(128)
#undef GC_ATT2F
#undef GC_ATT2
#undef GC_ATT2I
  return hipGetLastError();
}

hipError_t launch_attention(hipStream_t s, const float* qkv, float* o, float* part_o, float* part_ml,
                            int M, int B, int D, int H, int S, bool out_s16, const int* tile_chunk_start,
                            const int* union_idx, const unsigned* mask_bits, int n_tiles, bool feat16,
                            const int* items, int n_items) {
  const int os = out_s16 ? 1 : 0;
  if (H < 1 || D % H || S < 1) return hipErrorInvalidValue;
  const int dh = D / H;
  if ((dh == 128 && H > 4) || H > 8) return hipErrorInvalidValue;
  if (items && (S != 1 || n_items < 8 || n_items % 8 || out_s16)) return hipErrorInvalidValue;
  if (!items) n_items = 0;
  dim3 grid(items ? n_items : n_tiles, S, B), block(64 * H);
  if (dh == 32)
    hipLaunchKernelGGL((gc_attention_kernel<32>), grid, block, 0, s, qkv, o, part_o, part_ml, M, B, D, S, os,
                       tile_chunk_start, union_idx, mask_bits, feat16 ? 1 : 0, items, n_items);
  else if (dh == 64)
    hipLaunchKernelGGL((gc_attention_kernel<64>), grid, block, 0, s, qkv, o, part_o, part_ml, M, B, D, S, os,
                       tile_chunk_start, union_idx, mask_bits, feat16 ? 1 : 0, items, n_items);
  else if (dh == 128)
    hipLaunchKernelGGL((gc_attention_kernel<128>), grid, block, 0, s, qkv, o, part_o, part_ml, M, B, D, S, os,
                       tile_chunk_start, union_idx, mask_bits, feat16 ? 1 : 0, items, n_items);
  else
    return hipErrorInvalidValue;
  return hipGetLastError();
}

__global__ __launch_bounds__(256) void gc_finite_check_kernel(const float* __restrict__ p, size_t n,
                                                               unsigned* __restrict__ counter) {
  auto nonfinite = [](float v) { return (__builtin_bit_cast(unsigned, v) & 0x7f800000u) == 0x7f800000u; };
  unsigned bad = 0;
  const size_t n4 = n / 4;
  for (size_t i = (size_t)blockIdx.x * 256 + threadIdx.x; i < n4; i += (size_t)gridDim.x * 256) {
    const f32x4 v = ld4(p + 4 * i);
#pragma unroll
    for (int e = 0; e < 4; ++e) bad |= nonfinite(v[e]);
  }
  if (blockIdx.x == 0 && threadIdx.x < (n & 3)) bad |= nonfinite(p[4 * n4 + threadIdx.x]);
  if (__any(bad != 0) && (threadIdx.x & 63) == 0) atomicAdd(counter, 1u);
}

hipError_t launch_finite_check(hipStream_t s, const float* p, size_t n, unsigned* counter) {
  const int grid = (int)std::min<size_t>((n / 4 + 255) / 256 + 1, 1024);
  hipLaunchKernelGGL(gc_finite_check_kernel, dim3(grid), dim3(256), 0, s, p, n, counter);
  return hipGetLastError();
}

__global__ __launch_bounds__(256) void gc_pack_full_kernel(const float* __restrict__ grid_struct,
                                                            const float* __restrict__ feats, int G,
                                                            int B, int c_in, int kp,
                                                            float* __restrict__ xp) {
  const size_t total = (size_t)G * B * kp;
  for (size_t i = (size_t)blockIdx.x * 256 + threadIdx.x; i < total; i += (size_t)gridDim.x * 256) {
    const size_t row = i / kp;
    const int c = (int)(i - row * kp);
    float v = 0.f;
    if (c < 3)
      v = grid_struct[(row / B) * 3 + c];
    else if (c < 3 + c_in)
      v = feats[row * c_in + (c - 3)];
    xp[i] = v;
  }
}

__global__ __launch_bounds__(256) void gc_write_noisy_kernel(const float* __restrict__ x,
                                                              const int* __restrict__ slots, int rows,
                                                              int c_out, int kp, float scale,
                                                              float* __restrict__ xp) {
  const size_t total = (size_t)rows * c_out;
  for (size_t i = (size_t)blockIdx.x * 256 + threadIdx.x; i < total; i += (size_t)gridDim.x * 256) {
    const size_t row = i / c_out;
    const int c = (int)(i - row * c_out);
    xp[row * kp + 3 + slots[c]] = scale * x[i];
  }
}

__device__ __forceinline__ void put_noisy(const NoisyWrite& nw, size_t i, float v) {
  const size_t row = i / nw.c_out;
  const int c = (int)(i - row * nw.c_out);
  if (nw.xn) nw.xn[row * nw.ldn + c] = nw.scale * v;
  else nw.xp[row * nw.kp + 3 + nw.slots[c]] = nw.scale * v;
}

__global__ __launch_bounds__(256) void gc_write_noisy_compact_kernel(const float* __restrict__ x, int rows, int c_out,
                                                                      int ldn, float scale, float* __restrict__ xn) {
  const size_t total = (size_t)rows * c_out;
  for (size_t i = (size_t)blockIdx.x * 256 + threadIdx.x; i < total; i += (size_t)gridDim.x * 256) {
    const size_t row = i / c_out;
    xn[row * ldn + (i - row * c_out)] = scale * x[i];
  }
}

__global__ __launch_bounds__(256) void gc_zero_slots_kernel(const int* __restrict__ slots, int rows, int c_out, int kp,
                                                             float* __restrict__ xp) {
  const size_t total = (size_t)rows * c_out;
  for (size_t i = (size_t)blockIdx.x * 256 + threadIdx.x; i < total; i += (size_t)gridDim.x * 256) {
    const size_t row = i / c_out;
    xp[row * kp + 3 + slots[i - row * c_out]] = 0.f;
  }
}

__global__ __launch_bounds__(256) void gc_scale_kernel(const float* __restrict__ src, float a, size_t n,
                                                        float* __restrict__ dst, NoisyWrite nw) {
  for (size_t i = (size_t)blockIdx.x * 256 + threadIdx.x; i < n; i += (size_t)gridDim.x * 256) {
    const float v = a * src[i];
    dst[i] = v;
    if (nw.xp || nw.xn) put_noisy(nw, i, v);
  }
}

__global__ __launch_bounds__(256) void gc_dpm_first_kernel(const float* __restrict__ y,
                                                            const float* __restrict__ x, float c_out,
                                                            float c_skip, float a_mid, size_t n,
                                                            float* __restrict__ den,
                                                            float* __restrict__ mid, NoisyWrite nw) {
  for (size_t i = (size_t)blockIdx.x * 256 + threadIdx.x; i < n; i += (size_t)gridDim.x * 256) {
    const float xv = x[i];
    const float d = y[i] * c_out + xv * c_skip;
    den[i] = d;
    const float m = a_mid * xv + (1.0f - a_mid) * d;
    mid[i] = m;
    if (nw.xp || nw.xn) put_noisy(nw, i, m);
  }
}

__global__ __launch_bounds__(256) void gc_dpm_second_kernel(const float* __restrict__ y,
                                                             const float* __restrict__ xmid,
                                                             float c_out, float c_skip, float a_next,
                                                             size_t n, float* __restrict__ x, NoisyWrite nw) {
  for (size_t i = (size_t)blockIdx.x * 256 + threadIdx.x; i < n; i += (size_t)gridDim.x * 256) {
    const float md = y[i] * c_out + xmid[i] * c_skip;
    const float v = a_next * x[i] + (1.0f - a_next) * md;
    x[i] = v;
    if (nw.xp || nw.xn) put_noisy(nw, i, v);
  }
}

__global__ __launch_bounds__(256) void gc_affine_rows_kernel(const float* __restrict__ src,
                                                              const float* __restrict__ cond,
                                                              int cond_stride, size_t items, int B,
                                                              int w, float* __restrict__ out, int round16, int h16) {
  const size_t total = items * B * w;
  for (size_t i = (size_t)blockIdx.x * 256 + threadIdx.x; i < total; i += (size_t)gridDim.x * 256) {
    const size_t row = i / w;
    const int c = (int)(i - row * w);
    const size_t item = row / B;
    const int b = (int)(row - item * B);
    const float* cs = cond + (size_t)b * cond_stride;
    const float v = src[item * w + c] * cs[c] + cs[w + c];
    if (h16) as_h16(out)[i] = (_Float16)v;
    else out[i] = r16_if(v, round16);
  }
}

static int ew_grid(size_t n) {
  size_t g = (n + 255) / 256;
  return (int)(g > 2048 ? 2048 : (g ? g : 1));
}

hipError_t launch_pack_full(hipStream_t s, const float* grid_struct, const float* feats, int G, int B,
                            int c_in, int kp, float* xp) {
  hipLaunchKernelGGL(gc_pack_full_kernel, dim3(ew_grid((size_t)G * B * kp)), dim3(256), 0, s,
                     grid_struct, feats, G, B, c_in, kp, xp);
  return hipGetLastError();
}

hipError_t launch_write_noisy(hipStream_t s, const float* x, const int* slots, int rows, int c_out,
                              int kp, float scale, float* xp) {
  hipLaunchKernelGGL(gc_write_noisy_kernel, dim3(ew_grid((size_t)rows * c_out)), dim3(256), 0, s, x,
                     slots, rows, c_out, kp, scale, xp);
  return hipGetLastError();
}

hipError_t launch_write_noisy_compact(hipStream_t s, const float* x, int rows, int c_out, int ldn, float scale, float* xn) {
  hipLaunchKernelGGL(gc_write_noisy_compact_kernel, dim3(ew_grid((size_t)rows * c_out)), dim3(256), 0, s, x, rows, c_out, ldn,
                     scale, xn);
  return hipGetLastError();
}

hipError_t launch_zero_slots(hipStream_t s, const int* slots, int rows, int c_out, int kp, float* xp) {
  hipLaunchKernelGGL(gc_zero_slots_kernel, dim3(ew_grid((size_t)rows * c_out)), dim3(256), 0, s, slots, rows, c_out, kp, xp);
  return hipGetLastError();
}

hipError_t launch_affine_rows(hipStream_t s, const float* src, const float* cond, int cond_stride,
                              int items, int B, int w, float* out, bool round16, bool h16) {
  hipLaunchKernelGGL(gc_affine_rows_kernel, dim3(ew_grid((size_t)items * B * w)), dim3(256), 0, s, src,
                     cond, cond_stride, (size_t)items, B, w, out, round16 ? 1 : 0, h16 ? 1 : 0);
  return hipGetLastError();
}

hipError_t launch_scale(hipStream_t s, const float* src, float a, size_t n, float* dst, const NoisyWrite& nw) {
  hipLaunchKernelGGL(gc_scale_kernel, dim3(ew_grid(n)), dim3(256), 0, s, src, a, n, dst, nw);
  return hipGetLastError();
}

hipError_t launch_dpm_first(hipStream_t s, const float* y, const float* x, float c_out, float c_skip,
                            float a_mid, size_t n, float* den, float* mid, const NoisyWrite& nw) {
  hipLaunchKernelGGL(gc_dpm_first_kernel, dim3(ew_grid(n)), dim3(256), 0, s, y, x, c_out, c_skip,
                     a_mid, n, den, mid, nw);
  return hipGetLastError();
}

hipError_t launch_dpm_second(hipStream_t s, const float* y, const float* xmid, float c_out,
                             float c_skip, float a_next, size_t n, float* x, const NoisyWrite& nw) {
  hipLaunchKernelGGL(gc_dpm_second_kernel, dim3(ew_grid(n)), dim3(256), 0, s, y, xmid, c_out, c_skip,
                     a_next, n, x, nw);
  return hipGetLastError();
}

__global__ __launch_bounds__(256) void gc_rollout_advance_kernel(
    const float* __restrict__ old_feats, const float* __restrict__ sample, const float* __restrict__ forcings,
    const int* __restrict__ kind, const int* __restrict__ src, const int* __restrict__ sidx,
    const float* __restrict__ a, const float* __restrict__ b, int rows, int c_in, int c_out, int n_forcing,
    float* __restrict__ new_feats) {
// ... 175 lines not shown
```

### gencast-flax-nnx_amd/csrc/gc_kernels_decl.inc

```
namespace GC_KERNELS_NS {

enum KernelClass : int {
  KC_COND = 0,
  KC_PACK,
  KC_MLP,
  KC_SEGSUM,
  KC_ROWOP,
  KC_GEMM_QKV,
  KC_ATTN,
  KC_ATTN_COMBINE,
  KC_GEMM_OUT,
  KC_GEMM_FFW1,
  KC_GEMM_FFW2,
  KC_GEMM_NODE,
  KC_NOISE,
  KC_COUNT
};

constexpr int kTileM = 32;
constexpr int kCondDim = 16;

struct Segment {
  const float* ptr;
  const int* index;
  const float* affine;
  int width;
  int ld;
  int bcast;
};

struct AddTerm {
  const float* ptr;
  const int* index;
};

struct MlpArgs {
  Segment seg[3];
  int nseg;
  AddTerm add[3];
  int nadd;
  int rows;
  int B;
  int hidden;
  const float* w1t;
  int ldw1;
  const float* b1;
  const float* w2t;
  const float* b2;
  int n_out;
  int n_out_pad;
  int do_ln;
  const float* cond;
  int cond_stride;
  const float* residual;
  float* out;
  int ldo;
  int f16;
  const float* w1f;
  int k1f;
  const float* w2f;
  const float* ones;
  const float* zeros;
  int round16;
  int round_out;
  int a16;
  int seg0_f32;
  int out_f32;
  int f32w;
  int tri;
};
bool mlp_runs_weight_streaming(const MlpArgs& a);

hipError_t launch_cond(hipStream_t s, const float* sigma_dev, float sigma_scalar, int B,
                       const float* w0t, const float* b0, const float* w1t, const float* b1,
                       int nfreq, int nhid, float base_period,
                       const float* wc_all, const float* bc_all, int total, float* cond_vec,
                       float* cond_out);

constexpr int kMaxSigmaList = 96;
struct SigmaList { float v[kMaxSigmaList]; };
hipError_t launch_cond_multi(hipStream_t s, const SigmaList& sl, int ncalls, int B, const float* w0t,
                             const float* b0, const float* w1t, const float* b1, int nfreq, int nhid,
                             float base_period, const float* wc_all, const float* bc_all, int total,
                             float* cond_out);

hipError_t launch_mlp(hipStream_t s, const MlpArgs& a);
bool mlp_pair_supported(const MlpArgs& a, const MlpArgs& b);
hipError_t launch_mlp_pair(hipStream_t s, const MlpArgs& a, const MlpArgs& b);

hipError_t launch_segsum(hipStream_t s, const float* src, const int* rowptr, const int* eids,
                         int n_items, int n_edges, int B, int width, float* out, bool round16 = false,
                         bool h16 = false ,
                         float norm = 0.f );

struct GemmArgs {
  const float* a;
  int lda;
  int a_f32;
  const float* att_po;
  const float* att_pml;
  int att_S, att_B, att_H, att_DH;
  const int* att_tiles;
  const float* wt;
  int ldw;
  int rows, n;
  int k_slice;
  int splits;
  const float* bias;
  int act;
  float* out;
  int ldo;
  int round16;
  int a16;
  void* kv16;
  int kv_d;
  int out_f32;
  int f32w;
};
hipError_t launch_gemm(hipStream_t s, int cls, const GemmArgs& g, int splits, int epi, bool f16);
hipError_t launch_gemm_ws(hipStream_t s, int cls, const GemmArgs& g, int mt, int splits, int epi);
#ifdef GC_STAMPS
hipError_t set_gemm_ws_stamp_buffer(unsigned long long* p);
#endif

struct FfwArgs {
  const float* a;
  int rows, d, f;
  const float* w1f;
  const float* b1;
  const float* w2f;
  float* out;
  int round16;
  int a16;
  unsigned long long* stamps;
  int f32w;
};
hipError_t launch_ffw_fused(hipStream_t s, const FfwArgs& g);

struct RowFuse {
  float* x;
  const float* bias;
  const float* cond;
  int cond_stride;
  int B;
  float* h;
  int round16;
};
hipError_t launch_gemm_rowop(hipStream_t s, int cls, const GemmArgs& g, const RowFuse& f);
#ifdef GC_STAMPS
hipError_t set_gemm_rowop_stamp_buffer(unsigned long long* p);
#endif

hipError_t launch_rowop(hipStream_t s, float* x, const float* bias, const float* partials, int n_slabs,
                        int rows, int d, int B, const float* cond, int cond_stride, float* h,
                        int h_s16 ,
                        bool round16 = false, bool h16 = false );

hipError_t launch_attention(hipStream_t s, const float* qkv, float* o, float* part_o, float* part_ml,
                            int M, int B, int D, int H, int S, bool out_s16,
                            const int* tile_chunk_start, const int* union_idx, const unsigned* mask_bits,
                            int n_tiles, bool feat16 = false,
                            const int* items = nullptr , int n_items = 0);
hipError_t launch_attention_v2(hipStream_t s, const float* qkv, const void* kv16, float* o, float* part_o,
                               float* part_ml, int M, int B, int D, int H, int S, const int* tile_chunk_start,
                               const int* union_idx, const unsigned* mask_bits, int n_tiles,
                               int max_chunks_per_tile, bool feat16,
                               bool h16 = false ,
                               const int* items = nullptr ,
                               int n_items = 0);
#ifdef GC_STAMPS
hipError_t set_attention_stamp_buffer(unsigned long long* p);
#endif

hipError_t launch_pack_full(hipStream_t s, const float* grid_struct, const float* feats, int G, int B,
                            int c_in, int kp, float* xp);
hipError_t launch_write_noisy(hipStream_t s, const float* x, const int* slots, int rows, int c_out,
                              int kp, float scale, float* xp);
hipError_t launch_write_noisy_compact(hipStream_t s, const float* x, int rows, int c_out, int ldn, float scale, float* xn);
hipError_t launch_zero_slots(hipStream_t s, const int* slots, int rows, int c_out, int kp, float* xp);
hipError_t launch_affine_rows(hipStream_t s, const float* src, const float* cond, int cond_stride,
                              int items, int B, int w, float* out, bool round16 = false,
                              bool h16 = false );
hipError_t launch_finite_check(hipStream_t s, const float* p, size_t n, unsigned* counter);
constexpr int kItemPieces = 4;
struct NoisyWrite {
  const int* slots = nullptr;
  int c_out = 1, kp = 0;
  float scale = 0.f;
  float* xp = nullptr;
  float* xn = nullptr;
  int ldn = 0;
  bool active() const { return xp != nullptr || xn != nullptr; }
};
hipError_t launch_scale(hipStream_t s, const float* src, float a, size_t n, float* dst, const NoisyWrite& nw = NoisyWrite());
hipError_t launch_rollout_advance(hipStream_t s, const float* old_feats, const float* sample, const float* forcings,
                                  const int* kind, const int* src, const int* sidx, const float* a, const float* b,
                                  int rows, int c_in, int c_out, int n_forcing, float* new_feats);
hipError_t launch_dpm_first(hipStream_t s, const float* y, const float* x, float c_out, float c_skip,
                            float a_mid, size_t n, float* den, float* mid, const NoisyWrite& nw = NoisyWrite());
hipError_t launch_dpm_second(hipStream_t s, const float* y, const float* xmid, float c_out,
                             float c_skip, float a_next, size_t n, float* x, const NoisyWrite& nw = NoisyWrite());

constexpr int kLossMaxBlocks = 2048;
constexpr int kLossMaxGroups = 64;
constexpr size_t kLossMaxLds = 32 * 1024;
int loss_reduce_blocks(int G, int B, int c_out);
hipError_t launch_loss_noisy(hipStream_t s, const float* t, const float* nz, const float* sigma, const int* slots, int rows,
                             int B, int c_out, int kp, float* x, float* xp);
hipError_t launch_loss_reduce(hipStream_t s, const float* y, const float* t, const float* nz, const float* x,
                              const float* sigma, const float* node_w, int G, int B, int c_out, double* part, float* den);
hipError_t launch_loss_finish(hipStream_t s, const double* part, int blocks, const float* sigma, const float* chan_w,
                              const int* chan_group, const float* group_w, int B, int c_out, int n_groups, float* loss,
                              float* per_group);

hipError_t launch_noise_normals(hipStream_t s, float* out, size_t count, unsigned long long key,
                                unsigned long long stream);
hipError_t launch_noise_synthesis(hipStream_t s, const float* leg, const float* ctab, const float* stab,
                                  const float* coef, float* f, int L, int n_lat, int n_lon, int N,
                                  const float* base, float scale, float* out);

const char* kernel_class_name(int cls);

}
```

### gencast-flax-nnx_amd/csrc/gc_sampler.hip

```cpp
#include "gc_handle.h"

namespace gci {

int guard_enqueue(gc_handle* h, const float* p, size_t n) {
  if (!make_route(h).f16) return GC_OK;
  int rc = launch(h, gc::KC_PACK, [&] { return gc::launch_finite_check(h->stream, p, n, h->d_nonfinite); });
  if (rc) return rc;
  GC_HIP(h, hipMemcpyAsync(h->h_nonfinite, h->d_nonfinite, sizeof(unsigned), hipMemcpyDeviceToHost, h->stream));
  return GC_OK;
}
bool guard_tripped(gc_handle* h) {
  if (*h->h_nonfinite == h->nonfinite_seen) return false;
  h->nonfinite_seen = *h->h_nonfinite;
  return true;
}

float f_c_in(float s) { return 1.0f / std::sqrt(s * s + 1.0f); }
float f_c_out(float s) { return s / std::sqrt(s * s + 1.0f); }
float f_c_skip(float s) { return 1.0f / (s * s + 1.0f); }

int noise_field(gc_handle* h, const float* base, float scale, float* out) {
  if (h->nz_L == 0) return fail(h, GC_ERR_STATE, "gc_noise_set_tables has not been called");
  const int N = h->cfg.batch * h->cfg.c_out;
  const size_t ncoef = (size_t)2 * h->nz_L * h->nz_L * N;
  const unsigned long long stream = h->nz_stream++;
  int rc = launch(h, gc::KC_NOISE, [&] { return gc::launch_noise_normals(h->stream, h->d_nz_coef, ncoef, h->nz_key, stream); });
  if (rc) return rc;
  return launch(h, gc::KC_NOISE, [&] {
    return gc::launch_noise_synthesis(h->stream, h->d_nz_leg, h->d_nz_cos, h->d_nz_sin, h->d_nz_coef, h->d_nz_f,
                                      h->nz_L, h->nz_lat, h->nz_lon, N, base, scale, out);
  });
}

int sampler_body(gc_handle* h, const float* sigmas, int n, int skip_dead, const std::vector<float>& call_sigma,
                 bool multi, int* calls_out) {
  const gc_config& c = h->cfg;
  const int rows = h->hg.G * c.batch;
  const size_t ne = (size_t)rows * c.c_out;
  hipStream_t s = h->stream;
  int rc, calls = 0;
  const size_t cond_call = (size_t)c.batch * h->cond_total;
  const bool churn = !h->churn_rates.empty();
  h->embed_cache_live = true;
  struct CacheOff { gc_handle* h; ~CacheOff() { h->embed_cache_live = false; } } cache_off{h};
  const Route route = make_route(h);
  const bool cache = route.embed_cache;
  if (cache) {
    if ((rc = launch(h, gc::KC_PACK, [&] { return gc::launch_zero_slots(s, h->d_slots, rows, c.c_out, h->kp, h->d_xp); }))) return rc;
    gc::GemmArgs ga{};
    ga.a = h->d_xp; ga.lda = h->kp; ga.a_f32 = 1; ga.ldw = h->kp; ga.rows = rows; ga.n = c.latent_size; ga.k_slice = h->kp;
    ga.bias = nullptr; ga.act = 0; ga.out = h->d_pstat; ga.ldo = c.latent_size; ga.round16 = 0; ga.out_f32 = 1;
    ga.wt = route.f16 ? h->w1st_s : h->w1st_t;
    if ((rc = launch(h, gc::KC_GEMM_NODE, [&] { return gc::launch_gemm(s, gc::KC_GEMM_NODE, ga, 1, 0, route.f16); }))) return rc;
    ++h->embed_cache_samples;
  }
  if (route.edge_terms) {
    if (!multi || h->terms.call_slot.size() != call_sigma.size() ||
        std::memcmp(h->terms.sigmas.data(), call_sigma.data(), call_sigma.size() * sizeof(float)))
      return fail(h, GC_ERR_INTERNAL, "sampler: the edge-term cache was built for another noise-level list");
    ++h->edge_term_samples;
  }
  auto noisy_write = [&](float sigma_next_call) {
    gc::NoisyWrite nw;
    nw.slots = h->d_slots; nw.c_out = c.c_out; nw.kp = h->kp; nw.scale = f_c_in(std::max(sigma_next_call, 1e-6f));
    if (cache) { nw.xn = h->d_xn; nw.ldn = h->nwp; }
    else nw.xp = h->d_xp;
    return nw;
  };
  auto churned = [&](int i) { return churn && i < n && h->churn_rates[i] > 0.f; };
  bool written = false;
  {
    const gc::NoisyWrite nw = (n > 0 && !churned(0)) ? noisy_write(sigmas[0]) : gc::NoisyWrite();
    if ((rc = launch(h, gc::KC_PACK, [&] { return gc::launch_scale(s, h->d_noise, sigmas[0], ne, h->d_sx, nw); })))
      return rc;
    written = nw.active();
  }
  if (multi) {
    gc::SigmaList sl{};
    for (size_t i = 0; i < call_sigma.size(); ++i) sl.v[i] = call_sigma[i];
    if ((rc = launch(h, gc::KC_COND, [&] {
           return gc::launch_cond_multi(s, sl, (int)call_sigma.size(), c.batch, h->d_nw0t, h->d_nb0, h->d_nw1t,
                                        h->d_nb1, c.noise_num_frequencies, c.noise_hidden, c.noise_base_period,
                                        h->d_wc_all, h->d_bc_all, h->cond_total, h->d_cond_all);
         })))
      return rc;
  }
  auto denoise = [&](const float* x, float sigma) -> int {
    const float ss = std::max(sigma, 1e-6f);
    if (!written) {
      int r = launch(h, gc::KC_PACK, [&] {
        return cache ? gc::launch_write_noisy_compact(s, x, rows, c.c_out, h->nwp, f_c_in(ss), h->d_xn)
                     : gc::launch_write_noisy(s, x, h->d_slots, rows, c.c_out, h->kp, f_c_in(ss), h->d_xp);
      });
      if (r) return r;
    }
    written = false;
    const float* ready = nullptr;
    if (multi) {
      if (calls >= (int)call_sigma.size() || call_sigma[calls] != ss)
        return fail(h, GC_ERR_INTERNAL, "sampler: noise-level list out of step with the loop");
      ready = h->d_cond_all + (size_t)calls * cond_call;
    }
    h->term_slot = route.edge_terms ? h->terms.call_slot[calls] : -1;
    ++calls;
    return forward(h, ss, ready);
  };
  for (int i = 0; i < n; ++i) {
    float sg = sigmas[i];
    const float sn = sigmas[i + 1];
    if (churn && h->churn_rates[i] > 0.f) {
      const float s_new = sg * (1.0f + h->churn_rates[i]);
      const float extra = std::sqrt(std::max(s_new * s_new - sg * sg, 0.0f)) * h->churn_inflation;
      if ((rc = noise_field(h, h->d_sx, extra, h->d_sx))) return rc;
      sg = s_new;
    }
    const float sm = std::sqrt(sg * sn);
    if ((rc = denoise(h->d_sx, sg))) return rc;
    const float ss = std::max(sg, 1e-6f);
    const float a_mid = sm / sg;
    {
      const bool mid_call = (sn != 0.0f) || !skip_dead;
      const gc::NoisyWrite nw = mid_call ? noisy_write(sm) : gc::NoisyWrite();
      if ((rc = launch(h, gc::KC_PACK, [&] {
             return gc::launch_dpm_first(s, h->d_y, h->d_sx, f_c_out(ss), f_c_skip(ss), a_mid, ne,
                                         h->d_sden, h->d_smid, nw);
           })))
        return rc;
      written = nw.active();
    }
    if (sn == 0.0f) {
      if (!skip_dead && (rc = denoise(h->d_smid, sm))) return rc;
      GC_HIP(h, hipMemcpyAsync(h->d_sx, h->d_sden, ne * sizeof(float), hipMemcpyDeviceToDevice, s));
      written = false;
      continue;
    }
    if ((rc = denoise(h->d_smid, sm))) return rc;
    const float sms = std::max(sm, 1e-6f);
    const float a_next = sn / sg;
    {
      const gc::NoisyWrite nw = (i + 1 < n && !churned(i + 1)) ? noisy_write(sigmas[i + 1]) : gc::NoisyWrite();
      if ((rc = launch(h, gc::KC_PACK, [&] {
             return gc::launch_dpm_second(s, h->d_y, h->d_smid, f_c_out(sms), f_c_skip(sms), a_next, ne,
                                          h->d_sx, nw);
           })))
        return rc;
      written = nw.active();
    }
  }
  *calls_out = calls;
  return GC_OK;
}

int run_sampler(gc_handle* h, const float* sigmas, int n, int skip_dead, gc_sample_stats* stats) {
  const gc_config& c = h->cfg;
  const size_t ne = (size_t)h->hg.G * c.batch * c.c_out;
  hipStream_t s = h->stream;
  int rc, calls = 0;
  const unsigned long long stream0 = h->nz_stream;
  const bool churn = !h->churn_rates.empty();
  if (churn && (int)h->churn_rates.size() != n)
    return fail(h, GC_ERR_INVALID_ARGUMENT, "gc_set_churn was given a schedule of another length than this sample");
  std::vector<float> call_sigma;
  for (int i = 0; i < n; ++i) {
    float sg = sigmas[i];
    if (churn && h->churn_rates[i] > 0.f) sg = sg * (1.0f + h->churn_rates[i]);
    call_sigma.push_back(std::max(sg, 1e-6f));
    const float sn = sigmas[i + 1];
    if (sn != 0.0f || !skip_dead) call_sigma.push_back(std::max(std::sqrt(sg * sn), 1e-6f));
  }
  const bool multi = (int)call_sigma.size() <= gc::kMaxSigmaList;
  const size_t cond_call = (size_t)c.batch * h->cond_total;
  if (multi && call_sigma.size() * cond_call > h->cond_all_cap) {
    if ((rc = dev_alloc(h, &h->d_cond_all, call_sigma.size() * cond_call))) return rc;
    h->cond_all_cap = call_sigma.size() * cond_call;
  }
  if ((rc = multi ? ensure_edge_terms(h, call_sigma) : drop_edge_terms(h))) return rc;

  const bool eligible = h->use_graphs && multi && !churn && h->prof_cls < 0 && h->debug_layer_limit < 0 &&
                        h->debug_stop_layer < 0;
  gc_handle::SampleGraph* sg = nullptr;
  if (eligible) {
    const Route r = make_route(h);
    for (auto& g : h->sample_graphs)
      if (g.skip_dead == skip_dead && g.noise == h->d_noise && g.route.f16 == r.f16 && g.feat16 == h->feat16 && g.route.st16 == r.st16 &&
          (int)g.sigmas.size() == n + 1 && !std::memcmp(g.sigmas.data(), sigmas, (n + 1) * sizeof(float)))
        sg = &g;
    if (!sg) {
      if (h->sample_graphs.size() >= 8) {
        size_t lru = 0;
        for (size_t i = 1; i < h->sample_graphs.size(); ++i)
          if (h->sample_graphs[i].last_use < h->sample_graphs[lru].last_use) lru = i;
        destroy_sample_graph(h->sample_graphs[lru]);
        h->sample_graphs.erase(h->sample_graphs.begin() + lru);
      }
      gc_handle::SampleGraph g;
      g.sigmas.assign(sigmas, sigmas + n + 1);
      g.skip_dead = skip_dead; g.noise = h->d_noise; g.route = r; g.feat16 = h->feat16;
      g.last_use = ++h->graph_clock;
      h->sample_graphs.push_back(g);
      sg = nullptr;
    } else {
      sg->last_use = ++h->graph_clock;
    }
  }
  GC_HIP(h, hipEventRecord(h->ev0, s));
  static std::mutex capture_mutex;
  auto launch_exec = [&](gc_handle::SampleGraph* g) -> int {
    std::unique_lock<std::mutex> launch_lock(capture_mutex, std::defer_lock);
    if (h->graph_serialize) launch_lock.lock();
    const int i = g->exec2 ? g->next : 0;
    hipGraphExec_t ex = i ? g->exec2 : g->exec;
    if (!g->done[i]) GC_HIP(h, hipEventCreateWithFlags(&g->done[i], hipEventDisableTiming));
    else GC_HIP(h, hipEventSynchronize(g->done[i]));
    GC_HIP(h, hipGraphLaunch(ex, s));
    GC_HIP(h, hipEventRecord(g->done[i], s));
    g->next = i ^ 1;
    return GC_OK;
  };
  if (sg && sg->exec) {
    if ((rc = launch_exec(sg))) return rc;
    calls = sg->calls;
    h->launches_last_call = sg->launches_per_call;
    h->route = h->last_route = sg->route;
    if (sg->route.edge_terms) ++h->edge_term_samples;
    ++h->graph_replays;
  } else if (sg) {
    const int64_t l0 = h->launch_count;
    auto say = [&](const char* what) { if (h->graph_verbose) { std::fprintf(stderr, "[gc graph] %s\n", what); std::fflush(stderr); } };
    hipGraph_t graph = nullptr;
    hipGraphExec_t exec = nullptr, exec2 = nullptr;
    {
      std::lock_guard<std::mutex> capture_lock(capture_mutex);
      say("begin capture");
      GC_HIP(h, hipStreamBeginCapture(s, hipStreamCaptureModeThreadLocal));
      rc = sampler_body(h, sigmas, n, skip_dead, call_sigma, multi, &calls);
      const hipError_t e_end = hipStreamEndCapture(s, &graph);
      say("end capture");
      if (rc) {
        if (graph) (void)hipGraphDestroy(graph);
        return rc;
      }
      if (e_end != hipSuccess || !graph) return fail(h, GC_ERR_HIP, std::string("hipStreamEndCapture: ") + hipGetErrorString(e_end));
      hipError_t e_inst = hipGraphInstantiate(&exec, graph, nullptr, nullptr, 0);
      if (e_inst == hipSuccess) e_inst = hipGraphInstantiate(&exec2, graph, nullptr, nullptr, 0);
      if (e_inst != hipSuccess) {
        if (exec) (void)hipGraphExecDestroy(exec);
        (void)hipGraphDestroy(graph);
        return fail(h, GC_ERR_HIP, std::string("hipGraphInstantiate: ") + hipGetErrorString(e_inst));
      }
      say("instantiated");
    }
    sg->graph = graph; sg->exec = exec; sg->exec2 = exec2; sg->calls = calls; sg->next = 0;
    sg->launches = h->launch_count - l0;
    sg->launches_per_call = h->launches_last_call;
    sg->route = h->last_route;
    ++h->graph_captures;
    if ((rc = launch_exec(sg))) return rc;
    say("launched");
    ++h->graph_replays;
  } else if ((rc = sampler_body(h, sigmas, n, skip_dead, call_sigma, multi, &calls))) {
    return rc;
  }
  GC_HIP(h, hipEventRecord(h->ev1, s));
  h->has_sample = true;
  if (make_route(h).f16) {
    if ((rc = guard_enqueue(h, h->d_sx, ne))) return rc;
    h->last_sigmas.assign(sigmas, sigmas + n + 1);
    h->last_skip_dead = skip_dead;
    h->guard_pending = true;
    h->last_stream0 = stream0;
    h->last_noise = h->d_noise;
  }
  if (stats) {
    GC_HIP(h, hipEventSynchronize(h->ev1));
    float ms = 0.f;
    GC_HIP(h, hipEventElapsedTime(&ms, h->ev0, h->ev1));
    stats->denoiser_calls = calls;
    stats->device_ms = ms;
  }
  return GC_OK;
}

int resolve_guard(gc_handle* h) {
  GC_HIP(h, hipStreamSynchronize(h->stream));
  if (!h->guard_pending) return GC_OK;
  h->guard_pending = false;
  if (!guard_tripped(h)) return GC_OK;
  ++h->range_fallbacks;
  h->in_fallback = true;
  const unsigned long long stream_end = h->nz_stream;
  h->nz_stream = h->last_stream0;
  const std::vector<float> sig = h->last_sigmas;
  float* const noise_next = h->d_noise;
  h->d_noise = h->last_noise;
  int rc = run_sampler(h, sig.data(), (int)sig.size() - 1, h->last_skip_dead, nullptr);
  h->d_noise = noise_next;
  h->nz_stream = stream_end;
  h->in_fallback = false;
  if (rc) return rc;
  GC_HIP(h, hipStreamSynchronize(h->stream));
  return GC_OK;
}

void destroy_sample_graph(gc_handle::SampleGraph& g) {
  for (hipEvent_t& e : g.done)
    if (e) { (void)hipEventSynchronize(e); (void)hipEventDestroy(e); e = nullptr; }
  if (g.exec) (void)hipGraphExecDestroy(g.exec);
  if (g.exec2) (void)hipGraphExecDestroy(g.exec2);
  if (g.graph) (void)hipGraphDestroy(g.graph);
  g.exec = g.exec2 = nullptr;
  g.graph = nullptr;
}

void drop_sample_graphs(gc_handle* h) {
  for (auto& g : h->sample_graphs) destroy_sample_graph(g);
  h->sample_graphs.clear();
}

int loss_eval(gc_handle* h, int e, const float* sig, bool draw_noise, bool want_den) {
  const gc_config& c = h->cfg;
  const int G = h->hg.G, B = c.batch, ng = h->loss_groups;
  hipStream_t s = h->stream;
  int rc;
  if (draw_noise) {
    if ((rc = noise_field(h, nullptr, 1.0f, h->d_noise))) return rc;
    h->has_noise = true;
  }
  if ((rc = launch(h, gc::KC_PACK, [&] {
         return gc::launch_loss_noisy(s, h->d_targets, h->d_noise, sig, h->d_slots, G * B, B, c.c_out, h->kp, h->d_lx, h->d_xp);
       })))
    return rc;
  float* const sigma_own = h->d_sigma;
  h->d_sigma = const_cast<float*>(sig);
  rc = forward(h, -1.0f);
  h->d_sigma = sigma_own;
  if (rc) return rc;
  if ((rc = launch(h, gc::KC_PACK, [&] {
// ... 12 lines not shown
```

Baseline: 788.5 calls/s.

## Fuse row tails into MLP epilogues: first-layer LN, decoder MLP, DPM update

```diff
diff --git a/gencast-flax-nnx_amd/csrc/gc_api.hip b/gencast-flax-nnx_amd/csrc/gc_api.hip
--- a/gencast-flax-nnx_amd/csrc/gc_api.hip
+++ b/gencast-flax-nnx_amd/csrc/gc_api.hip
@@ -108,6 +108,7 @@
   h->attn_items = !off("GC_TUNE_ATTN_ITEMS");
   h->mlp_pair = !off("GC_TUNE_MLP_PAIR");
   h->edge_terms = !off("GC_TUNE_EDGE_TERMS");
+  h->row_tails = !off("GC_TUNE_ROW_TAILS");
   h->a16 = !off("GC_TUNE_A16");
   h->graph_serialize = on("GC_TUNE_GRAPH_SERIALIZE");
   h->graph_verbose = on("GC_TUNE_GRAPH_VERBOSE");
@@ -830,6 +831,7 @@
   else if (n == "m2g_fused_sum") *value = h->last_route.m2g_fused ? 1 : 0;
   else if (n == "embed_cache") *value = h->embed_cache_samples;
   else if (n == "edge_term_samples") *value = h->edge_term_samples;
+  else if (n == "row_tails") *value = h->row_tails_last;
   else if (n == "edge_term_cache_bytes") *value = h->terms.ready ? h->terms.bytes : 0;
   else if (n == "graph_replays") *value = h->graph_replays;
   else if (n == "graph_captures") *value = h->graph_captures;
diff --git a/gencast-flax-nnx_amd/csrc/gc_forward.hip b/gencast-flax-nnx_amd/csrc/gc_forward.hip
--- a/gencast-flax-nnx_amd/csrc/gc_forward.hip
+++ b/gencast-flax-nnx_amd/csrc/gc_forward.hip
@@ -26,6 +26,7 @@
   r.m2g_fused = h->m2g_fuse_sum && h->hg.m2g_tri && h->hidden_layers == 1 && streams;
   r.embed_cache = h->embed_cache_live && h->embed_cache_ready && !h->feat16 && h->hidden_layers == 1 && streams;
   r.edge_terms = h->embed_cache_live && h->terms.ready && edge_terms_possible(h) && r.f16;
+  r.row_tails = h->row_tails && r.f16 && !h->feat16 && h->hidden_layers == 1 && h->cfg.latent_size == 256 && D == 256;
   return r;
 }
 
@@ -50,6 +51,7 @@
   bool round_out = true;
   bool seg0_f32 = false, out_f32 = false;
   bool tri = false;
+  gc::MlpTail tail;
   MlpCall& segments(std::initializer_list<gc::Segment> l) { for (const auto& s : l) seg[nseg++] = s; return *this; }
   MlpCall& add_terms(std::initializer_list<gc::AddTerm> l) { for (const auto& t : l) add[nadd++] = t; return *this; }
 };
@@ -87,6 +89,7 @@
   a.seg0_f32 = c.seg0_f32 ? 1 : 0;
   a.out_f32 = c.out_f32 ? 1 : 0;
   a.tri = c.tri ? 1 : 0;
+  a.tail = c.tail;
   if (c.tri && !gc::mlp_runs_weight_streaming(a))
     return fail(h, GC_ERR_INTERNAL, "the triple-sum epilogue exists in the weight-streaming MLP kernel only");
   return GC_OK;
@@ -333,14 +336,27 @@
                                   h->g2m_agg_norm);
        })))
     return rc;
-  if ((rc = run_mlp(h, h->g2m_mesh, mlp_call({seg(m0, nullptr, nullptr, L, L, 0), seg(h->d_agg1, nullptr, nullptr, L, L, 0)},
-                                             g.M * B, B, h->d_x, L, m0))))
-    return rc;
-  if (!paired && (rc = run_mlp(h, h->g2m_grid, node))) return rc;
-
-  const int MB = g.M * B;
   const int n_layers = (h->debug_layer_limit >= 0 && h->debug_layer_limit < c.num_layers)
                            ? h->debug_layer_limit : c.num_layers;
+  h->row_tails_last = 0;
+  bool row_tail = false;
+  {
+    MlpCall mesh = mlp_call({seg(m0, nullptr, nullptr, L, L, 0), seg(h->d_agg1, nullptr, nullptr, L, L, 0)}, g.M * B, B, h->d_x, L, m0);
+    gc::MlpArgs ma{};
+    if (r.row_tails && n_layers > 0) {
+      mesh.tail.kind = gc::TAIL_ROWPASS;
+      mesh.tail.cond = cond + h->layers[0].cond_attn;
+      mesh.tail.out = h->d_h;
+      if ((rc = build_mlp_args(h, h->g2m_mesh, mesh, &ma))) return rc;
+      row_tail = gc::mlp_tail_supported(ma);
+      if (!row_tail) mesh.tail = gc::MlpTail();
+    }
+    if ((rc = row_tail ? enqueue_mlp(h, ma) : run_mlp(h, h->g2m_mesh, mesh))) return rc;
+    if (row_tail) ++h->row_tails_last;
+  }
+  if (!paired && (rc = run_mlp(h, h->g2m_grid, node))) return rc;
+
+  const int MB = g.M * B;
   const float* pend_bias = nullptr;
   int pend_slabs = 0;
   auto rowop = [&](const float* bias, int slabs, int cond_off, float* hout) {
@@ -352,7 +368,7 @@
   const int* att_items = r.att_items ? h->d_att_items : nullptr;
   for (int i = 0; i < n_layers; ++i) {
     const DevLayer& ly = h->layers[i];
-    if ((rc = rowop(pend_bias, pend_slabs, ly.cond_attn, h->d_h))) return rc;
+    if (!(i == 0 && row_tail) && (rc = rowop(pend_bias, pend_slabs, ly.cond_attn, h->d_h))) return rc;
     if (stop_here(i, 0)) return GC_OK;
     if (r.v2) {
       gc::GemmArgs ga = mesh_gemm_args(h, h->d_h, D, true);
@@ -410,12 +426,28 @@
          return gc::launch_segsum(s, h->d_f1, h->d_m2g_ptr, h->d_m2g_eid, g.G, g.E2, B, L, h->d_agg2, h->feat16, r.st16);
        })))
     return rc;
-  if ((rc = run_mlp(h, h->m2g_grid, mlp_call({seg(h->d_g1, nullptr, nullptr, L, L, 0), seg(h->d_agg2, nullptr, nullptr, L, L, 0)},
-                                             g.G * B, B, h->d_g2, L, h->d_g1))))
-    return rc;
+  MlpCall grid = mlp_call({seg(h->d_g1, nullptr, nullptr, L, L, 0), seg(h->d_agg2, nullptr, nullptr, L, L, 0)}, g.G * B, B, h->d_g2, L, h->d_g1);
   MlpCall dec = mlp_call({seg(h->d_g2, nullptr, nullptr, L, L, 0)}, g.G * B, B, h->d_y, c.c_out);
   dec.ln = dec.cond = false; dec.out_f32 = true;
-  if ((rc = run_mlp(h, h->m2g_dec, dec))) return rc;
+  bool dec_tail = false;
+  if (r.row_tails) {
+    gc::MlpArgs ga{}, da{};
+    if ((rc = build_mlp_args(h, h->m2g_dec, dec, &da))) return rc;
+    gc::MlpTail t = h->post;
+    t.kind = gc::TAIL_MLP;
+    t.out = h->d_y; t.n_out = da.n_out;
+    t.w1f = da.w1f; t.b1 = da.b1; t.w2f = da.w2f; t.b2 = da.b2;
+    grid.tail = t;
+    if ((rc = build_mlp_args(h, h->m2g_grid, grid, &ga))) return rc;
+    dec_tail = da.k1f == 256 && da.hidden == 256 && da.n_out_pad == 128 && da.ldo == da.n_out && gc::mlp_tail_supported(ga);
+    if (dec_tail) {
+      if ((rc = enqueue_mlp(h, ga))) return rc;
+      h->row_tails_last += 1 + (t.post != gc::POST_NONE ? 1 : 0);
+      h->post_taken = t.post != gc::POST_NONE;
+    }
+    grid.tail = gc::MlpTail();
+  }
+  if (!dec_tail && ((rc = run_mlp(h, h->m2g_grid, grid)) || (rc = run_mlp(h, h->m2g_dec, dec)))) return rc;
   h->launches_last_call = h->launch_count - launches0;
   return GC_OK;
 }
diff --git a/gencast-flax-nnx_amd/csrc/gc_handle.h b/gencast-flax-nnx_amd/csrc/gc_handle.h
--- a/gencast-flax-nnx_amd/csrc/gc_handle.h
+++ b/gencast-flax-nnx_amd/csrc/gc_handle.h
@@ -38,6 +38,7 @@
   bool try_pair = false;
   bool embed_cache = false;
   bool edge_terms = false;
+  bool row_tails = false;
   bool ws(int n, int k, int splits) const { return (f16 || x32) && n % 128 == 0 && (k / splits) % 128 == 0; }
 };
 
@@ -183,6 +184,10 @@
   int term_slot = -1;
   const float* m0_cur = nullptr;
   int64_t edge_term_samples = 0;
+  bool row_tails = true;
+  int64_t row_tails_last = 0;
+  gc::MlpTail post;
+  bool post_taken = false;
   float *d_ones = nullptr, *d_zeros = nullptr;
   int hidden_layers = 1;
   float* d_mlp_tmp[2] = {nullptr, nullptr};
@@ -422,7 +427,7 @@
     hipEvent_t done[2] = {nullptr, nullptr};
     int next = 0;
     int calls = 0;
-    int64_t launches_per_call = 0, launches = 0;
+    int64_t launches_per_call = 0, launches = 0, row_tails = 0;
     uint64_t last_use = 0;
   };
   bool use_graphs = true;
diff --git a/gencast-flax-nnx_amd/csrc/gc_kernels.hip b/gencast-flax-nnx_amd/csrc/gc_kernels.hip
--- a/gencast-flax-nnx_amd/csrc/gc_kernels.hip
+++ b/gencast-flax-nnx_amd/csrc/gc_kernels.hip
@@ -530,11 +530,52 @@
   return r;
 }
 
+template <int NG>
+__device__ __forceinline__ void rowpass_ln_cond(const f32x4 (&v)[NG], int d, const f32x4 (&sc)[NG], const f32x4 (&of)[NG],
+                                                f32x4 (&o)[NG]) {
+#pragma clang fp contract(off)
+  float s1 = 0.f, s2 = 0.f;
+#pragma unroll
+  for (int i = 0; i < NG; ++i) {
+    s1 += ((v[i][0] + v[i][1]) + v[i][2]) + v[i][3];
+    const float q01 = i == 0 ? v[i][0] * v[i][0] + v[i][1] * v[i][1] : __builtin_fmaf(v[i][0], v[i][0], v[i][1] * v[i][1]);
+    s2 += (q01 + v[i][2] * v[i][2]) + v[i][3] * v[i][3];
+  }
+  s1 = wave_sum(s1);
+  s2 = wave_sum(s2);
+  const float mean = s1 / (float)d;
+  const float var = fmaxf(__builtin_fmaf(-mean, mean, s2 / (float)d), 0.f);
+  const float rstd = 1.0f / sqrtf(var + 1e-6f);
+#pragma unroll
+  for (int i = 0; i < NG; ++i)
+#pragma unroll
+    for (int e = 0; e < 4; ++e) o[i][e] = __builtin_fmaf((v[i][e] - mean) * rstd, sc[i][e], of[i][e]);
+}
+
+__device__ __forceinline__ void dpm_first_update(float y, float x, float c_out, float c_skip, float a_mid, float& den, float& mid) {
+  den = __builtin_fmaf(x, c_skip, y * c_out);
+  mid = __builtin_fmaf(a_mid, x, (1.0f - a_mid) * den);
+}
+__device__ __forceinline__ float dpm_second_update(float y, float xmid, float x, float c_out, float c_skip, float a_next) {
+  const float md = __builtin_fmaf(y, c_out, xmid * c_skip);
+  return __builtin_fmaf(a_next, x, (1.0f - a_next) * md);
+}
+__device__ __forceinline__ void put_noisy_at(const NoisyWrite& nw, size_t row, int c, float v) {
+  if (nw.xn) nw.xn[row * nw.ldn + c] = nw.scale * v;
+  else nw.xp[row * nw.kp + 3 + nw.slots[c]] = nw.scale * v;
+}
+__device__ __forceinline__ void put_noisy(const NoisyWrite& nw, size_t i, float v) {
+  const size_t row = i / nw.c_out;
+  put_noisy_at(nw, row, (int)(i - row * nw.c_out), v);
+}
+
 template <int NT1, int WM, int NWC>
 constexpr int mlp_ws_occ() { return NWC >= 8 ? (NT1 == 1 ? 4 : 2) : ((WM >= 2 || NT1 >= 4) ? 1 : 2); }
-template <int NT1, int NT2, int MT, int WM, int NWC, int NW2, int OCC, bool A16, bool F32, bool TERMS = false>
+template <int NT1, int NT2, int MT, int WM, int NWC, int NW2, int OCC, bool A16, bool F32, bool TERMS = false, int TAIL = TAIL_NONE>
 __device__ __forceinline__ void gc_mlp_ws_body(const MlpArgs& a, const int bid) {
   static_assert(!(A16 && F32), "one or the other");
+  static_assert(TAIL == TAIL_NONE || (NT1 == 1 && NT2 == 1 && MT == 1 && WM == 1 && NWC == 8 && NW2 == 8 && !A16 && !F32 && !TERMS),
+                "a tail: the 8-wave 32-row product form, f16x3, float32 arrays");
   static_assert(!TERMS || (!A16 && !F32 && (NT1 * 32 * NWC) % 256 == 0 && (32 * MT) % (4 * NWC) == 0), "terms form: f16x3, whole 1 KB rows per wave");
   extern __shared__ __attribute__((aligned(16))) float smem[];
   constexpr int HID = NT1 * 32 * NWC, NPAD = NT2 * 32 * NW2, BM = 32 * MT * WM, NTHR = 64 * NWC * WM;
@@ -980,6 +1021,10 @@
       rv[rr][j] = rs;
     }
   }
+  constexpr int TR = 4, TSTEPS = HID / 16;
+  constexpr size_t tcts = (size_t)TSTEPS * 512;
+  f32x4 twh[TR][1], twl[TR][1], vt[RW];
+  if constexpr (TAIL == TAIL_MLP) ws_ring_fill<1, TR>(twh, twl, a.tail.w1f + (size_t)wave * tcts + lane * 4, tcts, TSTEPS);
   __syncthreads();
 #pragma unroll
   for (int rr = 0; rr < RW; ++rr) {
@@ -1032,7 +1077,9 @@
 #pragma unroll
     for (int rr = 0; rr < RW; ++rr) {
       const int orow = row0 + rbase + rr;
-      if (orow >= a.rows) break;
+      if constexpr (TAIL == TAIL_NONE) {
+        if (orow >= a.rows) break;
+      }
       f32x4 sc = sc1, of = of1;
       if (a.cond && !(a.B == 1 && vec_io)) {
         const float* cs = a.cond + (size_t)(orow % a.B) * a.cond_stride;
@@ -1044,6 +1091,10 @@
           }
       }
       const f32x4 v = r16_c<RND>(r16_c<RND>(ln_affine(yv[rr][j], mean[rr], rstd[rr], sc, of)) + rv[rr][j]);
+      if constexpr (TAIL != TAIL_NONE) {
+        vt[rr] = v;
+        if (orow >= a.rows) continue;
+      }
       if (A16 && !a.out_f32) {
         if (vec_io) {
           sth4(as_h16(a.out) + (size_t)orow * a.ldo + c, v);
@@ -1062,13 +1113,119 @@
     }
   }
   });
+
+  if constexpr (TAIL == TAIL_ROWPASS) {
+    f32x4 tsc[RW], tof[RW];
+#pragma unroll
+    for (int rr = 0; rr < RW; ++rr) {
+      const float* cs = a.tail.cond + (size_t)((row0 + rbase + rr) % a.B) * a.cond_stride;
+      tsc[rr] = ld4(cs + 4 * lane);
+      tof[rr] = ld4(cs + n + 4 * lane);
+    }
+#pragma unroll
+    for (int rr = 0; rr < RW; ++rr) {
+      const int orow = row0 + rbase + rr;
+      if (orow >= a.rows) break;
+      const f32x4 xv[1] = {vt[rr]}, sc[1] = {tsc[rr]}, of[1] = {tof[rr]};
+      f32x4 o[1];
+      rowpass_ln_cond<1>(xv, n, sc, of, o);
+      st4(a.tail.out + (size_t)orow * n + 4 * lane, o[0]);
+    }
+  }
+  if constexpr (TAIL == TAIL_MLP) {
+    constexpr int NW2T = 4, LDT = 32 * NW2T + 4;
+#pragma unroll
+    for (int rr = 0; rr < RW; ++rr) store4_s16(region, (size_t)(rbase + rr), LDH, 4 * lane, vt[rr][0], vt[rr][1], vt[rr][2], vt[rr][3]);
+    __syncthreads();
+    f32x16 acc[1][1], accx[1][1];
+#pragma unroll
+    for (int q = 0; q < 16; ++q) {
+      acc[0][0][q] = 0.f;
+      accx[0][0][q] = 0.f;
+    }
+    const float* trow = region + r * LDH + hh * 4;
+    const int cbase = wave * 32 + 4 * hh;
+    {
+      const float* twf1 = a.tail.w1f + (size_t)wave * tcts + lane * 4;
+      int s = 0;
+#pragma unroll 1
+      for (int st = 0; st < TSTEPS; st += 8) {
+        ws_quad<1, 1, TR, 0, false, false>(acc, accx, twh, twl, trow, 32 * LDH, st, twf1, tcts, s, TSTEPS);
+        ws_quad<1, 1, TR, 0, false, false>(acc, accx, twh, twl, trow, 32 * LDH, st + 4, twf1, tcts, s, TSTEPS);
+      }
+    }
+    const bool p2 = wave < NW2T;
+    const float* twf2 = a.tail.w2f + (size_t)(p2 ? wave : 0) * tcts + lane * 4;
+    if (p2) ws_ring_fill<1, TR>(twh, twl, twf2, tcts, TSTEPS);
+    __syncthreads();
+#pragma unroll
+    for (int j = 0; j < 4; ++j) {
+      const f32x4 bv = ld4(a.tail.b1 + cbase + 8 * j);
+      float u[4];
+#pragma unroll
+      for (int e = 0; e < 4; ++e) u[e] = swish(hilo(acc[0][0][4 * j + e], accx[0][0][4 * j + e]) + bv[e]);
+      store4_s16(region, (size_t)r, LDH, cbase + 8 * j, u[0], u[1], u[2], u[3]);
+    }
+    __syncthreads();
+#pragma unroll
+    for (int q = 0; q < 16; ++q) {
+      acc[0][0][q] = 0.f;
+      accx[0][0][q] = 0.f;
+    }
+    {
+      int s = 0;
+#pragma unroll 1
+      for (int st = 0; st < (p2 ? TSTEPS : 0); st += 8) {
+        ws_quad<1, 1, TR, 0, false, false>(acc, accx, twh, twl, trow, 32 * LDH, st, twf2, tcts, s, TSTEPS);
+        ws_quad<1, 1, TR, 0, false, false>(acc, accx, twh, twl, trow, 32 * LDH, st + 4, twf2, tcts, s, TSTEPS);
+      }
+    }
+    __syncthreads();
+    if (p2) {
+#pragma unroll
+      for (int j = 0; j < 4; ++j) {
+        const f32x4 bv = ld4(a.tail.b2 + cbase + 8 * j);
+        f32x4 yq;
+#pragma unroll
+        for (int e = 0; e < 4; ++e) yq[e] = hilo(acc[0][0][4 * j + e], accx[0][0][4 * j + e]) + bv[e];
+        st4(region + r * LDT + cbase + 8 * j, yq);
+      }
+    }
+    __syncthreads();
+    const int tn = a.tail.n_out, post = a.tail.post;
+    const int orow0 = row0 + rbase;
+    const int live = (a.rows - orow0 < RW ? a.rows - orow0 : RW) * tn;
+    const float pc_out = a.tail.c_out, pc_skip = a.tail.c_skip, pa = a.tail.a;
+    const float* px = a.tail.x;
+    float* pden = a.tail.den;
+    float* pdst = a.tail.dst;
+    float* yout = a.tail.out;
+    const NoisyWrite nw = a.tail.nw;
+    for (int idx = lane; idx < live; idx += 64) {
+      const int rr = idx / tn, c = idx - rr * tn;
+      const float y = region[(rbase + rr) * LDT + c];
+      const size_t i = (size_t)orow0 * tn + idx;
+      yout[i] = y;
+      if (post == POST_NONE) continue;
+      float nv;
+      if (post == POST_DPM_FIRST) {
+        float d;
+        dpm_first_update(y, px[i], pc_out, pc_skip, pa, d, nv);
+        pden[i] = d;
+      } else {
+        nv = dpm_second_update(y, px[i], pdst[i], pc_out, pc_skip, pa);
+      }
+      pdst[i] = nv;
+      if (nw.xp || nw.xn) put_noisy_at(nw, (size_t)(orow0 + rr), c, nv);
+    }
+  }
 }
 
 template <int NT1, int NT2, int MT, int WM, int NWC = 4, int NW2 = NWC,
           int OCC = mlp_ws_occ<NT1, WM, NWC>() , bool A16 = false,
-          bool F32 = false, bool TERMS = false>
+          bool F32 = false, bool TERMS = false, int TAIL = TAIL_NONE>
 __global__ __launch_bounds__(64 * NWC * WM, OCC) void gc_mlp_ws_kernel(MlpArgs a) {
-  gc_mlp_ws_body<NT1, NT2, MT, WM, NWC, NW2, OCC, A16, F32, TERMS>(a, (int)blockIdx.x);
+  gc_mlp_ws_body<NT1, NT2, MT, WM, NWC, NW2, OCC, A16, F32, TERMS, TAIL>(a, (int)blockIdx.x);
 }
 
 template <int NT1, int NT2, int MT, int WM, int NWC = 4, int NW2 = NWC,
@@ -1106,6 +1263,9 @@
       if (a.nseg > 1 && a.seg[i].width % KCc) return hipErrorInvalidValue;
     }
   }
+  if (a.tail.kind != TAIL_NONE &&
+      !(NT1 == 1 && NT2 == 1 && MT == 1 && WM == 1 && NWC == 8 && NW2 == 8 && mlp_tail_supported(a)))
+    return hipErrorInvalidValue;
   int grid = (a.rows + BM - 1) / BM;
   if (a.tri) {
     if (a.rows % 3 || a.residual || a.ldo % 4 || a.n_out % 4 ||
@@ -1184,6 +1344,27 @@
   return hipGetLastError();
 }
 
+template <bool A16TU>
+static hipError_t launch_mlp_ws_tail(hipStream_t s, const MlpArgs& a) {
+  if constexpr (A16TU) return hipErrorInvalidValue;
+  else {
+    int grid = 0;
+    size_t lds = 0;
+    if (hipError_t e = mlp_ws_geometry<1, 1, 1, 1, 8, 8>(a, &grid, &lds)) return e;
+    constexpr int OCC = mlp_ws_occ<1, 1, 8>();
+    if (a.tail.kind == TAIL_ROWPASS) {
+      static DynLdsOnce once_r;
+      if (hipError_t e = once_r.ensure((const void*)gc_mlp_ws_kernel<1, 1, 1, 1, 8, 8, OCC, false, false, false, TAIL_ROWPASS>, (int)lds)) return e;
+      hipLaunchKernelGGL((gc_mlp_ws_kernel<1, 1, 1, 1, 8, 8, OCC, false, false, false, TAIL_ROWPASS>), dim3(grid), dim3(512), lds, s, a);
+    } else {
+      static DynLdsOnce once_m;
+      if (hipError_t e = once_m.ensure((const void*)gc_mlp_ws_kernel<1, 1, 1, 1, 8, 8, OCC, false, false, false, TAIL_MLP>, (int)lds)) return e;
+      hipLaunchKernelGGL((gc_mlp_ws_kernel<1, 1, 1, 1, 8, 8, OCC, false, false, false, TAIL_MLP>), dim3(grid), dim3(512), lds, s, a);
+    }
+    return hipGetLastError();
+  }
+}
+
 template <int NT1, int NT2, bool F16, int WM>
 static hipError_t launch_mlp_t(hipStream_t s, const MlpArgs& a) {
   const int hidden = NT1 * 128, n_pad = NT2 * 128, bm = 32 * WM;
@@ -1207,9 +1388,23 @@
   return nt1 == 4 && (nt2 == 4 || nt2 == 1);
 }
 
+bool mlp_tail_supported(const MlpArgs& a) {
+  const MlpTail& t = a.tail;
+  auto aligned16 = [](const void* p) { return p && (reinterpret_cast<size_t>(p) & 15) == 0; };
+  if (t.kind != TAIL_ROWPASS && t.kind != TAIL_MLP) return false;
+  if (kTuA16 || !mlp_runs_weight_streaming(a) || !a.f16 || a.f32w || a.a16 || a.round16 || a.round_out || a.tri || a.nseg == 0) return false;
+  if (a.hidden != 256 || a.n_out_pad != 256 || a.n_out != 256 || a.rows >= kMlpMt2Rows || a.B < 1 || !t.out) return false;
+  if (t.kind == TAIL_ROWPASS) return aligned16(t.cond) && aligned16(t.out) && a.cond_stride % 4 == 0 && t.post == POST_NONE;
+  if (!aligned16(t.w1f) || !aligned16(t.b1) || !aligned16(t.w2f) || !aligned16(t.b2) || t.n_out < 1 || t.n_out > 128) return false;
+  if (t.post == POST_NONE) return true;
+  if ((t.post != POST_DPM_FIRST && t.post != POST_DPM_SECOND) || !t.x || !t.dst || (t.post == POST_DPM_FIRST && !t.den)) return false;
+  return !t.nw.active() || (t.nw.c_out == t.n_out && (t.nw.xn || t.nw.slots));
+}
+
 hipError_t launch_mlp(hipStream_t s, const MlpArgs& a) {
   const int nt1 = a.hidden / 128, nt2 = a.n_out_pad / 128;
   if (a.hidden % 128 || a.n_out_pad % 128 || a.n_out_pad > a.hidden) return hipErrorInvalidValue;
+  if (a.tail.kind != TAIL_NONE) return mlp_tail_supported(a) ? launch_mlp_ws_tail<kTuA16>(s, a) : hipErrorInvalidValue;
   if (mlp_runs_weight_streaming(a)) {
     if (a.nseg == 0) {
       if (nt1 != 2 || nt2 != 2) return hipErrorInvalidValue;
@@ -1240,7 +1435,7 @@
   return ok(a) && ok(b) && a.hidden == b.hidden && a.f16 == b.f16 && a.f32w == b.f32w && a.a16 == b.a16;
 }
 hipError_t launch_mlp_pair(hipStream_t s, const MlpArgs& a, const MlpArgs& b) {
-  if (!mlp_pair_supported(a, b)) return hipErrorInvalidValue;
+  if (!mlp_pair_supported(a, b) || a.tail.kind != TAIL_NONE || b.tail.kind != TAIL_NONE) return hipErrorInvalidValue;
   if (a.hidden == 512) return launch_mlp_ws_pair_t<2, 2, 2, 1, 8, 8>(s, a, b);
   if (a.nseg == 0) return launch_mlp_ws_pair_t<1, 1, 1, 1, 8, 8, true>(s, a, b);
   return launch_mlp_ws_pair_t<1, 1, 1, 1, 8, 8>(s, a, b);
@@ -2750,7 +2945,6 @@
   const size_t slab = (size_t)rows * d;
   const float* cs = cond + (size_t)(row % B) * cond_stride;
   float4 v[2], scv[2], ofv[2];
-  float s1 = 0.f, s2 = 0.f;
   const float4 zero4 = make_float4(0.f, 0.f, 0.f, 0.f);
 #pragma unroll
   for (int i = 0; i < 2; ++i) {
@@ -2793,31 +2987,26 @@
         else *reinterpret_cast<float4*>(x + (size_t)row * d + c) = a;
       }
       v[i] = a;
-      s1 += a.x + a.y + a.z + a.w;
-      s2 += a.x * a.x + a.y * a.y + a.z * a.z + a.w * a.w;
     }
   }
   if (!h) return;
-  s1 = wave_sum(s1);
-  s2 = wave_sum(s2);
-  const float mean = s1 / (float)d;
-  const float var = fmaxf(s2 / (float)d - mean * mean, 0.f);
-  const float rstd = 1.0f / sqrtf(var + 1e-6f);
+  f32x4 xv[2], sc[2], of[2], o[2];
+#pragma unroll
+  for (int i = 0; i < 2; ++i) {
+    xv[i] = f32x4{v[i].x, v[i].y, v[i].z, v[i].w};
+    sc[i] = f32x4{scv[i].x, scv[i].y, scv[i].z, scv[i].w};
+    of[i] = f32x4{ofv[i].x, ofv[i].y, ofv[i].z, ofv[i].w};
+  }
+  rowpass_ln_cond<2>(xv, d, sc, of, o);
 #pragma unroll
   for (int i = 0; i < 2; ++i) {
     const int c = 4 * lane + 256 * i;
     if (c < d) {
-      const float4 sc = scv[i];
-      const float4 of = ofv[i];
-      float4 o;
-      o.x = (v[i].x - mean) * rstd * sc.x + of.x;
-      o.y = (v[i].y - mean) * rstd * sc.y + of.y;
-      o.z = (v[i].z - mean) * rstd * sc.z + of.z;
-      o.w = (v[i].w - mean) * rstd * sc.w + of.w;
-      if (round16) { o.x = r16(o.x); o.y = r16(o.y); o.z = r16(o.z); o.w = r16(o.w); }
-      if constexpr (H16) sth4(as_h16(h) + (size_t)row * d + c, f32x4{o.x, o.y, o.z, o.w});
-      else if (h_s16) store4_s16(h, (size_t)row, d, c, o.x, o.y, o.z, o.w);
-      else *reinterpret_cast<float4*>(h + (size_t)row * d + c) = o;
+      f32x4 t = o[i];
+      if (round16) { t[0] = r16(t[0]); t[1] = r16(t[1]); t[2] = r16(t[2]); t[3] = r16(t[3]); }
+      if constexpr (H16) sth4(as_h16(h) + (size_t)row * d + c, t);
+      else if (h_s16) store4_s16(h, (size_t)row, d, c, t[0], t[1], t[2], t[3]);
+      else st4(h + (size_t)row * d + c, t);
     }
   }
 }
@@ -3496,13 +3685,6 @@
   }
 }
 
-__device__ __forceinline__ void put_noisy(const NoisyWrite& nw, size_t i, float v) {
-  const size_t row = i / nw.c_out;
-  const int c = (int)(i - row * nw.c_out);
-  if (nw.xn) nw.xn[row * nw.ldn + c] = nw.scale * v;
-  else nw.xp[row * nw.kp + 3 + nw.slots[c]] = nw.scale * v;
-}
-
 __global__ __launch_bounds__(256) void gc_write_noisy_compact_kernel(const float* __restrict__ x, int rows, int c_out,
                                                                       int ldn, float scale, float* __restrict__ xn) {
   const size_t total = (size_t)rows * c_out;
@@ -3536,10 +3718,9 @@
                                                             float* __restrict__ den,
                                                             float* __restrict__ mid, NoisyWrite nw) {
   for (size_t i = (size_t)blockIdx.x * 256 + threadIdx.x; i < n; i += (size_t)gridDim.x * 256) {
-    const float xv = x[i];
-    const float d = y[i] * c_out + xv * c_skip;
+    float d, m;
+    dpm_first_update(y[i], x[i], c_out, c_skip, a_mid, d, m);
     den[i] = d;
-    const float m = a_mid * xv + (1.0f - a_mid) * d;
     mid[i] = m;
     if (nw.xp || nw.xn) put_noisy(nw, i, m);
   }
@@ -3550,8 +3731,7 @@
                                                              float c_out, float c_skip, float a_next,
                                                              size_t n, float* __restrict__ x, NoisyWrite nw) {
   for (size_t i = (size_t)blockIdx.x * 256 + threadIdx.x; i < n; i += (size_t)gridDim.x * 256) {
-    const float md = y[i] * c_out + xmid[i] * c_skip;
-    const float v = a_next * x[i] + (1.0f - a_next) * md;
+    const float v = dpm_second_update(y[i], xmid[i], x[i], c_out, c_skip, a_next);
     x[i] = v;
     if (nw.xp || nw.xn) put_noisy(nw, i, v);
   }
diff --git a/gencast-flax-nnx_amd/csrc/gc_kernels_decl.inc b/gencast-flax-nnx_amd/csrc/gc_kernels_decl.inc
--- a/gencast-flax-nnx_amd/csrc/gc_kernels_decl.inc
+++ b/gencast-flax-nnx_amd/csrc/gc_kernels_decl.inc
@@ -32,6 +32,35 @@
 struct AddTerm {
   const float* ptr;
   const int* index;
+};
+
+struct NoisyWrite {
+  const int* slots = nullptr;
+  int c_out = 1, kp = 0;
+  float scale = 0.f;
+  float* xp = nullptr;
+  float* xn = nullptr;
+  int ldn = 0;
+  bool active() const { return xp != nullptr || xn != nullptr; }
+};
+
+enum MlpTailKind : int { TAIL_NONE = 0, TAIL_ROWPASS = 1, TAIL_MLP = 2 };
+enum MlpTailPost : int { POST_NONE = 0, POST_DPM_FIRST = 1, POST_DPM_SECOND = 2 };
+struct MlpTail {
+  int kind = TAIL_NONE;
+  float* out = nullptr;
+  const float* cond = nullptr;
+  const float* w1f = nullptr;
+  const float* b1 = nullptr;
+  const float* w2f = nullptr;
+  const float* b2 = nullptr;
+  int n_out = 0;
+  int post = POST_NONE;
+  float c_out = 0.f, c_skip = 0.f, a = 0.f;
+  const float* x = nullptr;
+  float* den = nullptr;
+  float* dst = nullptr;
+  NoisyWrite nw;
 };
 
 struct MlpArgs {
@@ -68,7 +97,9 @@
   int out_f32;
   int f32w;
   int tri;
-};
+  MlpTail tail;
+};
+bool mlp_tail_supported(const MlpArgs& a);
 bool mlp_runs_weight_streaming(const MlpArgs& a);
 
 hipError_t launch_cond(hipStream_t s, const float* sigma_dev, float sigma_scalar, int B,
@@ -183,15 +214,6 @@
                               bool h16 = false );
 hipError_t launch_finite_check(hipStream_t s, const float* p, size_t n, unsigned* counter);
 constexpr int kItemPieces = 4;
-struct NoisyWrite {
-  const int* slots = nullptr;
-  int c_out = 1, kp = 0;
-  float scale = 0.f;
-  float* xp = nullptr;
-  float* xn = nullptr;
-  int ldn = 0;
-  bool active() const { return xp != nullptr || xn != nullptr; }
-};
 hipError_t launch_scale(hipStream_t s, const float* src, float a, size_t n, float* dst, const NoisyWrite& nw = NoisyWrite());
 hipError_t launch_rollout_advance(hipStream_t s, const float* old_feats, const float* sample, const float* forcings,
                                   const int* kind, const int* src, const int* sidx, const float* a, const float* b,
diff --git a/gencast-flax-nnx_amd/csrc/gc_sampler.hip b/gencast-flax-nnx_amd/csrc/gc_sampler.hip
--- a/gencast-flax-nnx_amd/csrc/gc_sampler.hip
+++ b/gencast-flax-nnx_amd/csrc/gc_sampler.hip
@@ -85,7 +85,7 @@
          })))
       return rc;
   }
-  auto denoise = [&](const float* x, float sigma) -> int {
+  auto denoise = [&](const float* x, float sigma, const gc::MlpTail& post, bool* post_done) -> int {
     const float ss = std::max(sigma, 1e-6f);
     if (!written) {
       int r = launch(h, gc::KC_PACK, [&] {
@@ -103,8 +103,22 @@
     }
     h->term_slot = route.edge_terms ? h->terms.call_slot[calls] : -1;
     ++calls;
-    return forward(h, ss, ready);
+    h->post = post;
+    h->post_taken = false;
+    const int r = forward(h, ss, ready);
+    *post_done = h->post_taken;
+    h->post = gc::MlpTail();
+    h->post_taken = false;
+    return r;
   };
+  auto dpm_post = [&](int kind, const float* x, float sigma_call, float a, float* den, float* dst, const gc::NoisyWrite& nw) {
+    gc::MlpTail p;
+    p.post = kind; p.c_out = f_c_out(sigma_call); p.c_skip = f_c_skip(sigma_call); p.a = a;
+    p.x = x; p.den = den; p.dst = dst; p.nw = nw;
+    return p;
+  };
+  const gc::MlpTail no_post;
+  bool post_done = false;
   for (int i = 0; i < n; ++i) {
     float sg = sigmas[i];
     const float sn = sigmas[i + 1];
@@ -115,13 +129,13 @@
       sg = s_new;
     }
     const float sm = std::sqrt(sg * sn);
-    if ((rc = denoise(h->d_sx, sg))) return rc;
     const float ss = std::max(sg, 1e-6f);
     const float a_mid = sm / sg;
     {
       const bool mid_call = (sn != 0.0f) || !skip_dead;
       const gc::NoisyWrite nw = mid_call ? noisy_write(sm) : gc::NoisyWrite();
-      if ((rc = launch(h, gc::KC_PACK, [&] {
+      if ((rc = denoise(h->d_sx, sg, dpm_post(gc::POST_DPM_FIRST, h->d_sx, ss, a_mid, h->d_sden, h->d_smid, nw), &post_done))) return rc;
+      if (!post_done && (rc = launch(h, gc::KC_PACK, [&] {
              return gc::launch_dpm_first(s, h->d_y, h->d_sx, f_c_out(ss), f_c_skip(ss), a_mid, ne,
                                          h->d_sden, h->d_smid, nw);
            })))
@@ -129,17 +143,17 @@
       written = nw.active();
     }
     if (sn == 0.0f) {
-      if (!skip_dead && (rc = denoise(h->d_smid, sm))) return rc;
+      if (!skip_dead && (rc = denoise(h->d_smid, sm, no_post, &post_done))) return rc;
       GC_HIP(h, hipMemcpyAsync(h->d_sx, h->d_sden, ne * sizeof(float), hipMemcpyDeviceToDevice, s));
       written = false;
       continue;
     }
-    if ((rc = denoise(h->d_smid, sm))) return rc;
     const float sms = std::max(sm, 1e-6f);
     const float a_next = sn / sg;
     {
       const gc::NoisyWrite nw = (i + 1 < n && !churned(i + 1)) ? noisy_write(sigmas[i + 1]) : gc::NoisyWrite();
-      if ((rc = launch(h, gc::KC_PACK, [&] {
+      if ((rc = denoise(h->d_smid, sm, dpm_post(gc::POST_DPM_SECOND, h->d_smid, sms, a_next, nullptr, h->d_sx, nw), &post_done))) return rc;
+      if (!post_done && (rc = launch(h, gc::KC_PACK, [&] {
              return gc::launch_dpm_second(s, h->d_y, h->d_smid, f_c_out(sms), f_c_skip(sms), a_next, ne,
                                           h->d_sx, nw);
            })))
@@ -221,6 +235,7 @@
     if ((rc = launch_exec(sg))) return rc;
     calls = sg->calls;
     h->launches_last_call = sg->launches_per_call;
+    h->row_tails_last = sg->row_tails;
     h->route = h->last_route = sg->route;
     if (sg->route.edge_terms) ++h->edge_term_samples;
     ++h->graph_replays;
@@ -253,6 +268,7 @@
     sg->graph = graph; sg->exec = exec; sg->exec2 = exec2; sg->calls = calls; sg->next = 0;
     sg->launches = h->launch_count - l0;
     sg->launches_per_call = h->launches_last_call;
+    sg->row_tails = h->row_tails_last;
     sg->route = h->last_route;
     ++h->graph_captures;
     if ((rc = launch_exec(sg))) return rc;
```

After: 799.9 calls/s, median of 6. 1.4% higher.
